# unitaryai/VTC

Measured on AMD Instinct MI355X. Metric: video-text pairs encoded/sec (config 3: 8-frame TimeSformer video + title + 5 comments, CAM) + 10k x 10k sim+R@K ms, higher is better.
Workload: dtype bf16 (video tower) + f16 (text tower blocks), fp32 accumulate; 1 GPU; configs/pretrained_clip_timesformer_comments_attention.jsonc PretrainedCLIP_TimeSformer_finaltf forward: 1024 pairs/GPU/step = 1024 videos (8 x 3 x 224 x 224) + 1024 titles + 5120 comments (77 tokens) + CAM + sim; pairs_per_gpu=1024, frames=8, text_tower=ragged: tokens after EOT are not computed, identical outputs, parallelism=dp1 (one process per GPU, no collective in the encode path)

## Files before the change

include/vtc_hip.h:

```cpp
#ifndef VTC_HIP_H
#define VTC_HIP_H

#include <stddef.h>
#include <stdint.h>

#ifdef __cplusplus
extern "C" {
#endif

enum { VTC_F32 = 0, VTC_BF16 = 1, VTC_U8 = 2 ,
       VTC_F16 = 3  };

enum { VTC_ACT_NONE = 0, VTC_ACT_NORMALIZE = 1, VTC_ACT_SQUASH = 2, VTC_ACT_TANH = 3,
       VTC_ACT_SUB_MEAN = 4, VTC_ACT_BN = 5 };

enum { VTC_SWEEP_F32 = 0,
       VTC_SWEEP_BF16X3 = 1,
       VTC_SWEEP_BF16 = 2,
       VTC_SWEEP_EXACT = 3 };

typedef struct {
  const float *ln1_g, *ln1_b;
  const void  *qkv_w;  const float *qkv_b;
  const void  *out_w;  const float *out_b;
  const float *ln2_g, *ln2_b;
  const void  *fc_w;   const float *fc_b;
  const void  *proj_w; const float *proj_b;
  const float *lnt_g, *lnt_b;
  const void  *tqkv_w; const float *tqkv_b;
  const void  *tout_w; const float *tout_b;
  const void  *tfc_w;  const float *tfc_b;
  const void  *qkv_wf;  const float *qkv_s,  *qkv_c;
  const void  *fc_wf;   const float *fc_s,   *fc_c;
  const void  *tqkv_wf; const float *tqkv_s, *tqkv_c;
} vtc_block_w;

enum { VTC_TOWER_NO_LN_FOLD = 1,
       VTC_TOWER_FULL_LAST_LAYER = 8,
       VTC_TOWER_NO_SPLITK = 16         };

typedef struct {
  int width, heads, layers, patch, grid, embed_dim, nframes;
  int variant;
  int flags;
  float pix_mean[3], pix_std[3];
  const void  *conv_w;
  const float *class_embedding;
  const float *pos;
  const float *temporal;
  const float *ln_pre_g, *ln_pre_b, *ln_post_g, *ln_post_b;
  const float *proj_t;
  const vtc_block_w *blocks;
} vtc_vision_w;

typedef struct {
  int width, heads, layers, ctx, vocab, embed_dim;
  int half_layers;
  int flags;
  const float *tok_emb;
  const float *pos;
  const float *ln_final_g, *ln_final_b;
  const float *proj_t;
  const vtc_block_w *blocks;
} vtc_text_w;

typedef struct {
  int width, heads, layers;
  int init_from_avg;
  int residual_activation;
  float squash_scale;
  const void  *final_linear;
  const float *mask_embedding;
  const vtc_block_w *blocks;
  const float *bn_mean, *bn_var;
  int flags;
} vtc_cam_w;
enum { VTC_CAM_NO_FUSED = 1 };

const char *vtc_last_error(void);
int vtc_abi_version(void);


size_t vtc_vision_workspace_bytes(const vtc_vision_w *w, int n_items, int frames, int dtype);
int vtc_vision_forward(const vtc_vision_w *w, const void *pixels, int pixel_dtype, int n_items, int frames,
                       float *out, void *ws, size_t ws_bytes, int dtype, void *stream);

size_t vtc_text_workspace_bytes(const vtc_text_w *w, int n_seq, int dtype);
int vtc_text_forward(const vtc_text_w *w, const int64_t *ids, int n_seq, float *out, void *ws, size_t ws_bytes,
                     int dtype, void *stream);

int vtc_text_forward2(const vtc_text_w *w, const int64_t *ids_a, int n_a, const int64_t *ids_b, int n_b, int ragged, float *out,
                      void *ws, size_t ws_bytes, int dtype, void *stream);

size_t vtc_text_ragged_workspace_bytes(const vtc_text_w *w, int n_seq, int total_rows, int dtype);
int vtc_text_forward_ragged(const vtc_text_w *w, const int64_t *ids, int n_seq, const int *seq_offsets, int total_rows,
                            float *out, void *ws, size_t ws_bytes, int dtype, void *stream);

size_t vtc_cam_workspace_bytes(const vtc_cam_w *w, int B, int nc, int dtype);
int vtc_cam_forward(const vtc_cam_w *w, const float *main_feats, const float *comm_feats, const int64_t *comments,
                    int ctx, int B, int nc, float *adapted, void *ws, size_t ws_bytes, int dtype, void *stream);
int vtc_cam_fused_gave_up(int device);

size_t vtc_cam_aux_workspace_bytes(const vtc_cam_w *w, int B, int nc, int na, int dtype);
int vtc_cam_forward_aux(const vtc_cam_w *w, const float *main_feats, const float *comm_feats, const int64_t *comments,
                        const float *aux, int ctx, int B, int nc, int na, float *adapted, void *ws, size_t ws_bytes, int dtype,
                        void *stream);

size_t vtc_feature_mlp_workspace_bytes(int n, int d);
int vtc_feature_mlp(const float *x, int n, int d, const float *w1, const float *b1, const float *w2, const float *b2, float *y,
                    void *ws, size_t ws_bytes, void *stream);


size_t vtc_resize_plan_bytes(int in_h, int in_w, int size);
int vtc_resize_plan(int in_h, int in_w, int size, void *plan_host, size_t bytes);
int vtc_resize_crop_u8(const unsigned char *frames, int n, int in_h, int in_w, int layout, const void *plan_dev, int size,
                       unsigned char *out, void *stream);

int vtc_normalize_rows(const float *x, float *out, int n, int d, void *stream);
int vtc_normalize_rows2(const float *x, float *outx, int nx, const float *y, float *outy, int ny, int d, int *flag, void *stream);
int vtc_mean_groups(const float *x, float *out, int n_groups, int group, int d, void *stream);
int vtc_pack_tokens(const int *tokens, const int *offsets, int n_seq, int ctx, int sot, int eot, int64_t *ids, void *stream);

int vtc_mean_head_groups(const float *a, const float *b, float *out, int n_groups, int group, int d, void *stream);
int vtc_segment_mean(const float *x, const int *offsets, float *out, int n_groups, int d, void *stream);
int vtc_nonfinite_flag(const float *x, size_t n, int *flag, void *stream);
int vtc_nonfinite_flag2(const float *x, size_t n, const float *y, size_t m, int *flag, void *stream);
int vtc_similarity(const float *v, const float *t, int nv, int nt, int d, const float *logit_scale, float *sim,
                   void *stream);

size_t vtc_clip_loss_workspace_bytes(int n);
int vtc_clip_loss(const float *sim, int n, float *loss, void *ws, size_t ws_bytes, void *stream);


size_t vtc_l2_topk_workspace_bytes(int n_gallery, int n_queries, int d, int precision, int rows_per_block);
int vtc_l2_topk(const float *gallery, const float *queries, int n_gallery, int n_queries, int d, int depth,
                int precision, int rows_per_block, int64_t *ids, float *dists, void *ws, size_t ws_bytes,
                void *stream);

size_t vtc_l2_topk_bidir_workspace_bytes(int n_a, int n_b, int d, int precision, int rows_per_block);
int vtc_l2_topk_bidir(const float *a, const float *b, int n_a, int n_b, int d, int depth, int precision, int rows_per_block,
                      int64_t *ids_b2a, float *dists_b2a, int64_t *ids_a2b, float *dists_a2b, void *ws, size_t ws_bytes,
                      void *stream);
int vtc_l2_sweep_row_block(void);
int vtc_l2_sweep_shard_supported(int n_total, int n_local, int depth);
size_t vtc_l2_sweep_shard_workspace_bytes(int n_total, int n_local, int d);
int vtc_l2_sweep_shard_rows(const float *a_all, const float *b_local, int n_total, int n_local, int d, int depth, int64_t *ids,
                            float *dists, unsigned *col_planes, int nblk_pad, void *ws, size_t ws_bytes, void *stream);
int vtc_l2_sweep_shard_cols(const float *b_all, const float *a_local, int n_total, int n_local, int d, int depth,
                            const unsigned *planes, int n_src, int nblk_pad, const int *src_base, int64_t *ids, float *dists,
                            void *ws, size_t ws_bytes, void *stream);
size_t vtc_l2_search_workspace_bytes(int n_gallery, int n_queries, int d, int depth);
int vtc_l2_search(const float *gallery, const float *queries, int n_gallery, int n_queries, int d, int depth, int64_t id_base,
                  int64_t *ids, float *dists, int *nonfinite, void *ws, size_t ws_bytes, void *stream);
int vtc_l2_search_masked(const float *gallery, const float *queries, const uint32_t *live, int n_gallery, int n_queries, int d, int depth,
                         int64_t id_base, int64_t *ids, float *dists, int *nonfinite, void *ws, size_t ws_bytes, void *stream);
int vtc_row_mask_pack(const uint8_t *flags, int n_rows, const uint32_t *and_mask, uint32_t *words, void *stream);
int vtc_l2_search_merge(const int64_t *ids_parts, const double *dists_parts, int n_parts, int n_queries, int depth, int64_t *ids,
                        float *dists, void *stream);
size_t vtc_l2_search_grouped_workspace_bytes(int n_gallery, int n_queries, int d, int depth);
int vtc_l2_search_grouped(const float *gallery, const float *queries, const uint32_t *live, const int32_t *groups, int n_gallery, int n_queries,
                          int d, int depth, int64_t id_base, int64_t *ids, int32_t *out_groups, float *dists, int *nonfinite, void *ws,
                          size_t ws_bytes, void *stream);
int vtc_l2_search_merge_grouped(const int64_t *ids_parts, const double *dists_parts, const int32_t *groups_parts, int n_parts, int n_queries,
                                int depth, int64_t *ids, int32_t *out_groups, float *dists, void *stream);
int vtc_recall_hits(const int64_t *ids, int n_queries, int depth, int64_t target_offset, const int *k_vals_host,
                    int nk, long long *hits, void *stream);
#define VTC_RECALL_NONFINITE (1ll << 40)
int vtc_l2_recall_bidir_supported(int n, int d);
size_t vtc_l2_recall_bidir_workspace_bytes(int n, int d);
int vtc_l2_recall_bidir(const float *a, const float *b, int n, int d, const int *k_vals_host, int nk, long long *hits_b_from_a,
                        long long *hits_a_from_b, void *ws, size_t ws_bytes, void *stream);
float vtc_l2_rank_kappa(int d);
size_t vtc_l2_rank_bidir_workspace_bytes(int n, int d, int rows_per_block, int reach_capacity);
int vtc_l2_rank_bidir(const float *a, const float *b, int n, int d, int rows_per_block, int reach_capacity, int64_t *rank_a,
                      int64_t *rank_b, int *nonfinite, void *ws, size_t ws_bytes, void *stream);
size_t vtc_l2_rank_shard_workspace_bytes(int n_total, int n_local, int d, int rows_per_block, int reach_capacity);
int vtc_l2_rank_shard(const float *a_all, const float *b_all, int n_total, int row_base, int n_local, int d, int rows_per_block,
                      int reach_capacity, int64_t *rank_a_local , int64_t *rank_b_part , int *nonfinite,
                      void *ws, size_t ws_bytes, void *stream);
size_t vtc_l2_rank_grouped_workspace_bytes(int n, int m, int d, int rows_per_block, int reach_capacity);
int vtc_l2_rank_grouped(const float *a, const float *b, const int *off, int n, int m, int d, int rows_per_block, int reach_capacity,
                        int64_t *rank_a , int64_t *rank_b , int *nonfinite, void *ws, size_t ws_bytes, void *stream);
size_t vtc_l2_rank_grouped_vunit_workspace_bytes(int n, int m, int d, int rows_per_block, int reach_capacity);
int vtc_l2_rank_grouped_vunit(const float *a, const float *b, const int *off, int n, int m, int d, int rows_per_block, int reach_capacity,
                              int64_t *rank_a , int64_t *rank_b , int64_t *rank_v , int *nonfinite, void *ws,
                              size_t ws_bytes, void *stream);
int vtc_l2_recall_shard_supported(int n_total, int n_local, int d);
int vtc_l2_recall_planes(const int *k_vals_host, int nk, int n_total);
int vtc_l2_recall_shard_rows(const float *a_all, const float *b_local, int n_total, int n_local, int row_base, int d,
                             const int *k_vals_host, int nk, long long *hits_b_from_a, unsigned *col_planes, int nblk_pad, void *ws,
                             size_t ws_bytes, void *stream);
int vtc_l2_recall_shard_cols(const float *b_all, const float *a_local, int n_total, int n_local, int row_base, int d,
                             const int *k_vals_host, int nk, const unsigned *planes, int n_src, int nblk_pad, const int *src_bounds,
                             long long *hits_a_from_b, void *ws, size_t ws_bytes, void *stream);
int vtc_recall_hits_pair(const int64_t *ids_a, const int64_t *ids_b, int n_queries, int depth, int64_t target_offset,
                         const int *k_vals_host, int nk, long long *hits_a, long long *hits_b, void *stream);

enum { VTC_EPI_STORE = 0,
       VTC_EPI_GELU = 1,
       VTC_EPI_RESID = 2 };
int vtc_gemm(const void *A, const void *W, const float *bias, void *out, int M, int N, int K, int dtype,
             int epilogue, int out_dtype, int skip_mod, void *stream);
size_t vtc_gemm_resid_layernorm_workspace_bytes(int M);
int vtc_gemm_resid_layernorm_supported(int M, int N, int K, int dtype);
int vtc_gemm_resid_layernorm(const void *A, const void *W, const float *bias, float *out, int M, int N, int K, int dtype,
                             int skip_mod, const float *ln_g, const float *ln_b, void *ln_out, void *ws, size_t ws_bytes,
                             void *stream);
int vtc_layernorm(const float *x, const float *g, const float *b, void *y, int rows, int width, int out_dtype,
                  const int *row_index, int row_mul, void *stream);
int vtc_attention(const void *qkv, void *out, float *cls_out, int n_seq, int L, int heads, int causal, int s2, int a0,
                  int a1, int a2, int a3, int pstride, int dtype, void *stream);

int vtc_single_query_attention(const void *qkv, const void *q, float *out, int n_out, int L, int heads, int s2, int a0, int a1, int a2,
                               int a3, int pstride, const int *eot, const int *offs, int ctx, int dtype, void *stream);

int vtc_transpose_f32(const float *x, float *y, int rows, int cols, void *stream);
int vtc_colsum_f32(const float *x, float *out, int rows, int cols, void *stream);
int vtc_layernorm_bwd(const float *x, const float *gamma, const float *dy, float *dx, float *dgamma, float *dbeta, int rows,
                      int width, int accumulate_dx, void *stream);
int vtc_attention_small_bwd(const float *qkv, const float *dout, float *dqkv, int n_seq, int L, int heads, void *stream);
int vtc_quickgelu(const float *x, const float *dy, float *out, size_t n, void *stream);
int vtc_normalize_rows_bwd(const float *x, const float *dy, float *dx, int n, int d, void *stream);
int vtc_clip_loss_bwd(const float *sim, int n, float *dsim, void *ws, size_t ws_bytes, void *stream);
int vtc_adam_step(float *p, const float *g, float *m, float *v, float *vmax, size_t n, float lr, float beta1, float beta2,
                  float eps, int step, int amsgrad, void *stream);
int vtc_axpby(float *out, const float *x, const float *y, float a, float b, size_t n, void *stream);
int vtc_scale_rows(float *x, const float *s, int rows, int d, int group, void *stream);

enum { VTC_PROF_GEMM_BF16 = 0, VTC_PROF_GEMM_F32 = 1, VTC_PROF_ATTN = 2, VTC_PROF_NORM = 3, VTC_PROF_EMBED = 4,
       VTC_PROF_TOPK = 5, VTC_PROF_NCLASS = 6 };
enum { VTC_PROF_REGION_OTHER = 0, VTC_PROF_REGION_ATTN = 1, VTC_PROF_REGION_MLP = 2, VTC_PROF_NREGION = 3 };
int vtc_prof_begin(void);
int vtc_prof_end(void *stream, double *ms, long long *launches, double *work);
int vtc_prof_end_regions(void *stream, double *ms, long long *launches, double *work);
int vtc_prof_end_records(void *stream, int max, int *n, int *cls, int *region, double *ms, double *work, int *tag);
long long vtc_debug_launch_count(void);

#ifdef __cplusplus
}
#endif
#endif
```

vtc_amd/_lib.py:

```python
from __future__ import annotations

import ctypes as C
import os

_HERE = os.path.dirname(os.path.abspath(__file__))
LIB_PATH = os.environ.get("VTC_HIP_LIB") or os.path.join(_HERE, "lib", "libvtc_hip.so")

VTC_F32, VTC_BF16, VTC_U8 = 0, 1, 2
ACT_NONE, ACT_NORMALIZE, ACT_SQUASH, ACT_TANH, ACT_SUB_MEAN, ACT_BN = 0, 1, 2, 3, 4, 5
SWEEP_F32, SWEEP_BF16X3, SWEEP_BF16, SWEEP_EXACT = 0, 1, 2, 3
EPI_STORE, EPI_GELU, EPI_RESID = 0, 1, 2
PROF_CLASSES = ("gemm_bf16", "gemm_f32", "attention", "norm", "embed", "topk")
PROF_REGIONS = ("other", "attn", "mlp")
VTC_F16 = 3
TOWER_NO_LN_FOLD, TOWER_FULL_LAST_LAYER, TOWER_NO_SPLITK = 1, 8, 16
CAM_NO_FUSED = 1
RECALL_NONFINITE = 1 << 40
ABI_VERSION = 7

vp, fp, ip = C.c_void_p, C.c_void_p, C.c_void_p


class BlockW(C.Structure):
    _fields_ = [(n, C.c_void_p) for n in (
        "ln1_g", "ln1_b", "qkv_w", "qkv_b", "out_w", "out_b", "ln2_g", "ln2_b", "fc_w", "fc_b", "proj_w", "proj_b",
        "lnt_g", "lnt_b", "tqkv_w", "tqkv_b", "tout_w", "tout_b", "tfc_w", "tfc_b",
        "qkv_wf", "qkv_s", "qkv_c", "fc_wf", "fc_s", "fc_c", "tqkv_wf", "tqkv_s", "tqkv_c")]


class VisionW(C.Structure):
    _fields_ = [("width", C.c_int), ("heads", C.c_int), ("layers", C.c_int), ("patch", C.c_int), ("grid", C.c_int),
                ("embed_dim", C.c_int), ("nframes", C.c_int), ("variant", C.c_int), ("flags", C.c_int),
                ("pix_mean", C.c_float * 3), ("pix_std", C.c_float * 3),
                ("conv_w", C.c_void_p), ("class_embedding", C.c_void_p), ("pos", C.c_void_p), ("temporal", C.c_void_p),
                ("ln_pre_g", C.c_void_p), ("ln_pre_b", C.c_void_p), ("ln_post_g", C.c_void_p), ("ln_post_b", C.c_void_p),
                ("proj_t", C.c_void_p), ("blocks", C.POINTER(BlockW))]


class TextW(C.Structure):
    _fields_ = [("width", C.c_int), ("heads", C.c_int), ("layers", C.c_int), ("ctx", C.c_int), ("vocab", C.c_int),
                ("embed_dim", C.c_int), ("half_layers", C.c_int), ("flags", C.c_int),
                ("tok_emb", C.c_void_p), ("pos", C.c_void_p), ("ln_final_g", C.c_void_p), ("ln_final_b", C.c_void_p),
                ("proj_t", C.c_void_p), ("blocks", C.POINTER(BlockW))]


class CamW(C.Structure):
    _fields_ = [("width", C.c_int), ("heads", C.c_int), ("layers", C.c_int), ("init_from_avg", C.c_int),
                ("residual_activation", C.c_int), ("squash_scale", C.c_float),
                ("final_linear", C.c_void_p), ("mask_embedding", C.c_void_p), ("blocks", C.POINTER(BlockW)),
                ("bn_mean", C.c_void_p), ("bn_var", C.c_void_p), ("flags", C.c_int)]


SIGNATURES = {
    "vtc_last_error": (C.c_char_p, []),
    "vtc_abi_version": (C.c_int, []),
    "vtc_vision_workspace_bytes": (C.c_size_t, [C.POINTER(VisionW), C.c_int, C.c_int, C.c_int]),
    "vtc_vision_forward": (C.c_int, [C.POINTER(VisionW), vp, C.c_int, C.c_int, C.c_int, fp, vp, C.c_size_t, C.c_int, vp]),
    "vtc_text_workspace_bytes": (C.c_size_t, [C.POINTER(TextW), C.c_int, C.c_int]),
    "vtc_text_forward": (C.c_int, [C.POINTER(TextW), ip, C.c_int, fp, vp, C.c_size_t, C.c_int, vp]),
    "vtc_text_forward2": (C.c_int, [C.POINTER(TextW), ip, C.c_int, ip, C.c_int, C.c_int, fp, vp, C.c_size_t, C.c_int, vp]),
    "vtc_text_ragged_workspace_bytes": (C.c_size_t, [C.POINTER(TextW), C.c_int, C.c_int, C.c_int]),
    "vtc_text_forward_ragged": (C.c_int, [C.POINTER(TextW), ip, C.c_int, ip, C.c_int, fp, vp, C.c_size_t, C.c_int, vp]),
    "vtc_cam_workspace_bytes": (C.c_size_t, [C.POINTER(CamW), C.c_int, C.c_int, C.c_int]),
    "vtc_cam_forward": (C.c_int, [C.POINTER(CamW), fp, fp, ip, C.c_int, C.c_int, C.c_int, fp, vp, C.c_size_t, C.c_int, vp]),
    "vtc_cam_fused_gave_up": (C.c_int, [C.c_int]),
    "vtc_cam_aux_workspace_bytes": (C.c_size_t, [C.POINTER(CamW), C.c_int, C.c_int, C.c_int, C.c_int]),
    "vtc_cam_forward_aux": (C.c_int, [C.POINTER(CamW), fp, fp, ip, fp, C.c_int, C.c_int, C.c_int, C.c_int, fp, vp, C.c_size_t, C.c_int,
                                      vp]),
    "vtc_feature_mlp_workspace_bytes": (C.c_size_t, [C.c_int, C.c_int]),
    "vtc_feature_mlp": (C.c_int, [fp, C.c_int, C.c_int, fp, fp, fp, fp, fp, vp, C.c_size_t, vp]),
    "vtc_resize_plan_bytes": (C.c_size_t, [C.c_int, C.c_int, C.c_int]),
    "vtc_resize_plan": (C.c_int, [C.c_int, C.c_int, C.c_int, vp, C.c_size_t]),
    "vtc_resize_crop_u8": (C.c_int, [vp, C.c_int, C.c_int, C.c_int, C.c_int, vp, C.c_int, vp, vp]),
    "vtc_normalize_rows": (C.c_int, [fp, fp, C.c_int, C.c_int, vp]),
    "vtc_normalize_rows2": (C.c_int, [fp, fp, C.c_int, fp, fp, C.c_int, C.c_int, vp, vp]),
    "vtc_mean_groups": (C.c_int, [fp, fp, C.c_int, C.c_int, C.c_int, vp]),
    "vtc_nonfinite_flag": (C.c_int, [fp, C.c_size_t, vp, vp]),
    "vtc_nonfinite_flag2": (C.c_int, [fp, C.c_size_t, fp, C.c_size_t, vp, vp]),
    "vtc_mean_head_groups": (C.c_int, [fp, fp, fp, C.c_int, C.c_int, C.c_int, vp]),
    "vtc_pack_tokens": (C.c_int, [vp, vp, C.c_int, C.c_int, C.c_int, C.c_int, vp, vp]),
    "vtc_single_query_attention": (C.c_int, [vp, vp, fp] + [C.c_int] * 9 + [vp, vp, C.c_int, C.c_int, vp]),
    "vtc_segment_mean": (C.c_int, [fp, ip, fp, C.c_int, C.c_int, vp]),
    "vtc_similarity": (C.c_int, [fp, fp, C.c_int, C.c_int, C.c_int, fp, fp, vp]),
    "vtc_clip_loss_workspace_bytes": (C.c_size_t, [C.c_int]),
    "vtc_clip_loss": (C.c_int, [fp, C.c_int, fp, vp, C.c_size_t, vp]),
    "vtc_l2_topk_workspace_bytes": (C.c_size_t, [C.c_int, C.c_int, C.c_int, C.c_int, C.c_int]),
    "vtc_l2_topk": (C.c_int, [fp, fp, C.c_int, C.c_int, C.c_int, C.c_int, C.c_int, C.c_int, ip, fp, vp, C.c_size_t, vp]),
    "vtc_l2_topk_bidir_workspace_bytes": (C.c_size_t, [C.c_int, C.c_int, C.c_int, C.c_int, C.c_int]),
    "vtc_l2_topk_bidir": (C.c_int, [fp, fp, C.c_int, C.c_int, C.c_int, C.c_int, C.c_int, C.c_int, ip, fp, ip, fp, vp, C.c_size_t, vp]),
    "vtc_l2_sweep_row_block": (C.c_int, []),
    "vtc_l2_sweep_shard_supported": (C.c_int, [C.c_int, C.c_int, C.c_int]),
    "vtc_l2_sweep_shard_workspace_bytes": (C.c_size_t, [C.c_int, C.c_int, C.c_int]),
    "vtc_l2_sweep_shard_rows": (C.c_int, [fp, fp, C.c_int, C.c_int, C.c_int, C.c_int, ip, fp, vp, C.c_int, vp, C.c_size_t, vp]),
    "vtc_l2_sweep_shard_cols": (C.c_int, [fp, fp, C.c_int, C.c_int, C.c_int, C.c_int, vp, C.c_int, C.c_int, vp, ip, fp, vp,
                                          C.c_size_t, vp]),
    "vtc_l2_search_workspace_bytes": (C.c_size_t, [C.c_int, C.c_int, C.c_int, C.c_int]),
    "vtc_l2_search": (C.c_int, [fp, fp, C.c_int, C.c_int, C.c_int, C.c_int, C.c_int64, ip, fp, ip, vp, C.c_size_t, vp]),
    "vtc_l2_search_masked": (C.c_int, [fp, fp, ip, C.c_int, C.c_int, C.c_int, C.c_int, C.c_int64, ip, fp, ip, vp, C.c_size_t, vp]),
    "vtc_row_mask_pack": (C.c_int, [vp, C.c_int, ip, ip, vp]),
    "vtc_l2_search_merge": (C.c_int, [ip, fp, C.c_int, C.c_int, C.c_int, ip, fp, vp]),
    "vtc_l2_search_grouped_workspace_bytes": (C.c_size_t, [C.c_int, C.c_int, C.c_int, C.c_int]),
    "vtc_l2_search_grouped": (C.c_int, [fp, fp, ip, ip, C.c_int, C.c_int, C.c_int, C.c_int, C.c_int64, ip, ip, fp, ip, vp, C.c_size_t, vp]),
    "vtc_l2_search_merge_grouped": (C.c_int, [ip, fp, ip, C.c_int, C.c_int, C.c_int, ip, ip, fp, vp]),
    "vtc_recall_hits": (C.c_int, [ip, C.c_int, C.c_int, C.c_int64, C.POINTER(C.c_int), C.c_int, vp, vp]),
    "vtc_recall_hits_pair": (C.c_int, [ip, ip, C.c_int, C.c_int, C.c_int64, C.POINTER(C.c_int), C.c_int, vp, vp, vp]),
    "vtc_l2_recall_bidir_supported": (C.c_int, [C.c_int, C.c_int]),
    "vtc_l2_recall_bidir_workspace_bytes": (C.c_size_t, [C.c_int, C.c_int]),
    "vtc_l2_recall_bidir": (C.c_int, [fp, fp, C.c_int, C.c_int, C.POINTER(C.c_int), C.c_int, ip, ip, vp, C.c_size_t, vp]),
    "vtc_l2_rank_kappa": (C.c_float, [C.c_int]),
    "vtc_l2_rank_bidir_workspace_bytes": (C.c_size_t, [C.c_int, C.c_int, C.c_int, C.c_int]),
    "vtc_l2_rank_bidir": (C.c_int, [fp, fp, C.c_int, C.c_int, C.c_int, C.c_int, ip, ip, ip, vp, C.c_size_t, vp]),
    "vtc_l2_rank_shard_workspace_bytes": (C.c_size_t, [C.c_int, C.c_int, C.c_int, C.c_int, C.c_int]),
    "vtc_l2_rank_shard": (C.c_int, [fp, fp, C.c_int, C.c_int, C.c_int, C.c_int, C.c_int, C.c_int, ip, ip, ip, vp, C.c_size_t, vp]),
    "vtc_l2_rank_grouped_workspace_bytes": (C.c_size_t, [C.c_int, C.c_int, C.c_int, C.c_int, C.c_int]),
    "vtc_l2_rank_grouped": (C.c_int, [fp, fp, ip, C.c_int, C.c_int, C.c_int, C.c_int, C.c_int, ip, ip, ip, vp, C.c_size_t, vp]),
    "vtc_l2_rank_grouped_vunit_workspace_bytes": (C.c_size_t, [C.c_int, C.c_int, C.c_int, C.c_int, C.c_int]),
    "vtc_l2_rank_grouped_vunit": (C.c_int, [fp, fp, ip, C.c_int, C.c_int, C.c_int, C.c_int, C.c_int, ip, ip, ip, ip, vp, C.c_size_t, vp]),
    "vtc_l2_recall_shard_supported": (C.c_int, [C.c_int, C.c_int, C.c_int]),
    "vtc_l2_recall_planes": (C.c_int, [C.POINTER(C.c_int), C.c_int, C.c_int]),
    "vtc_l2_recall_shard_rows": (C.c_int, [fp, fp, C.c_int, C.c_int, C.c_int, C.c_int, C.POINTER(C.c_int), C.c_int, ip, vp, C.c_int, vp, C.c_size_t, vp]),
    "vtc_l2_recall_shard_cols": (C.c_int, [fp, fp, C.c_int, C.c_int, C.c_int, C.c_int, C.POINTER(C.c_int), C.c_int, vp, C.c_int, C.c_int, vp, ip, vp,
                                           C.c_size_t, vp]),
    "vtc_gemm": (C.c_int, [vp, vp, fp, vp, C.c_int, C.c_int, C.c_int, C.c_int, C.c_int, C.c_int, C.c_int, vp]),
    "vtc_gemm_resid_layernorm_workspace_bytes": (C.c_size_t, [C.c_int]),
    "vtc_gemm_resid_layernorm_supported": (C.c_int, [C.c_int, C.c_int, C.c_int, C.c_int]),
    "vtc_gemm_resid_layernorm": (C.c_int, [vp, vp, fp, fp, C.c_int, C.c_int, C.c_int, C.c_int, C.c_int, fp, fp, vp, vp, C.c_size_t, vp]),
    "vtc_layernorm": (C.c_int, [fp, fp, fp, vp, C.c_int, C.c_int, C.c_int, ip, C.c_int, vp]),
    "vtc_prof_begin": (C.c_int, []),
    "vtc_prof_end": (C.c_int, [vp, C.POINTER(C.c_double), C.POINTER(C.c_longlong), C.POINTER(C.c_double)]),
    "vtc_prof_end_regions": (C.c_int, [vp, C.POINTER(C.c_double), C.POINTER(C.c_longlong), C.POINTER(C.c_double)]),
    "vtc_prof_end_records": (C.c_int, [vp, C.c_int, C.POINTER(C.c_int), C.POINTER(C.c_int), C.POINTER(C.c_int), C.POINTER(C.c_double),
                                       C.POINTER(C.c_double), C.POINTER(C.c_int)]),
    "vtc_debug_launch_count": (C.c_longlong, []),
    "vtc_attention": (C.c_int, [vp, vp, fp, C.c_int, C.c_int, C.c_int, C.c_int, C.c_int, C.c_int, C.c_int, C.c_int,
                                C.c_int, C.c_int, C.c_int, vp]),
    "vtc_transpose_f32": (C.c_int, [fp, fp, C.c_int, C.c_int, vp]),
    "vtc_colsum_f32": (C.c_int, [fp, fp, C.c_int, C.c_int, vp]),
    "vtc_layernorm_bwd": (C.c_int, [fp, fp, fp, fp, fp, fp, C.c_int, C.c_int, C.c_int, vp]),
    "vtc_attention_small_bwd": (C.c_int, [fp, fp, fp, C.c_int, C.c_int, C.c_int, vp]),
    "vtc_quickgelu": (C.c_int, [fp, fp, fp, C.c_size_t, vp]),
    "vtc_normalize_rows_bwd": (C.c_int, [fp, fp, fp, C.c_int, C.c_int, vp]),
    "vtc_clip_loss_bwd": (C.c_int, [fp, C.c_int, fp, vp, C.c_size_t, vp]),
    "vtc_adam_step": (C.c_int, [fp, fp, fp, fp, fp, C.c_size_t, C.c_float, C.c_float, C.c_float, C.c_float, C.c_int, C.c_int, vp]),
    "vtc_axpby": (C.c_int, [fp, fp, fp, C.c_float, C.c_float, C.c_size_t, vp]),
    "vtc_scale_rows": (C.c_int, [fp, fp, C.c_int, C.c_int, C.c_int, vp]),
}

_lib = None


def lib() -> C.CDLL:
    global _lib
    if _lib is None:
        if not os.path.exists(LIB_PATH):
            raise RuntimeError(
                f"libvtc_hip.so not found at {LIB_PATH}: build it with `python -c 'import __graft_entry__ as g; g.build()'` "
                "(or `make -C vtc_amd/csrc`).  vtc_amd has no CPU or PyTorch fallback.")
        l = C.CDLL(LIB_PATH)
        for name, (res, args) in SIGNATURES.items():
            f = getattr(l, name)
            f.restype, f.argtypes = res, args
        _lib = l
    return _lib


def check(rc: int, what: str):
    if rc != 0:
        msg = lib().vtc_last_error().decode("utf-8", "replace")
        raise RuntimeError(f"{what} failed: {msg}")
```

vtc_amd/csrc/common.h:

```cpp
#pragma once
#include <hip/hip_runtime.h>
#include <stdint.h>
#include <stdio.h>

#include "../../include/vtc_hip.h"

typedef unsigned short bf16_t;
typedef __attribute__((ext_vector_type(8))) short bf16x8;
typedef __attribute__((ext_vector_type(4))) short bf16x4;
typedef __attribute__((ext_vector_type(4))) float f32x4;
typedef __attribute__((ext_vector_type(16))) float f32x16;

#define VTC_WAVE 64

void vtc_count_launch();
#undef hipLaunchKernelGGL
#define hipLaunchKernelGGL(kernelName, numBlocks, numThreads, memPerBlock, streamId, ...)             \
  do {                                                                                              \
    vtc_count_launch();                                                                             \
    (kernelName)<<<(numBlocks), (numThreads), (memPerBlock), (streamId)>>>(__VA_ARGS__);            \
  } while (0)

void vtc_set_error(const char *fmt, ...);

#define VTC_CHECK(cond, ...)          \
  do {                                \
    if (!(cond)) {                    \
      vtc_set_error(__VA_ARGS__);     \
      return 1;                       \
    }                                 \
  } while (0)

#define VTC_LAUNCH_CHECK(name)                                                  \
  do {                                                                          \
    hipError_t e_ = hipGetLastError();                                          \
    if (e_ != hipSuccess) {                                                     \
      vtc_set_error("%s: launch failed: %s", name, hipGetErrorString(e_));      \
      return 1;                                                                 \
    }                                                                           \
  } while (0)

#define VTC_LAUNCH_CHECK2(fn, stage)                                                          \
  do {                                                                                        \
    hipError_t e_ = hipGetLastError();                                                        \
    if (e_ != hipSuccess) {                                                                   \
      vtc_set_error("%s %s: launch failed: %s", fn, stage, hipGetErrorString(e_));            \
      return 1;                                                                               \
    }                                                                                         \
  } while (0)

__device__ __forceinline__ bf16_t f2bf(float f) {
  __bf16 b = (__bf16)f;
  return __builtin_bit_cast(bf16_t, b);
}
__device__ __forceinline__ float bf2f(bf16_t b) {
  return __builtin_bit_cast(float, ((unsigned)b) << 16);
}

struct f16_t { unsigned short v; };
typedef __attribute__((ext_vector_type(8))) _Float16 f16x8;
__device__ __forceinline__ unsigned short f2h(float f) {
  _Float16 h = (_Float16)f;
  return __builtin_bit_cast(unsigned short, h);
}
__device__ __forceinline__ float h2f(unsigned short b) { return (float)__builtin_bit_cast(_Float16, b); }
template <typename T> __device__ __forceinline__ unsigned short cvt16(float f);
template <> __device__ __forceinline__ unsigned short cvt16<bf16_t>(float f) { return f2bf(f); }
template <> __device__ __forceinline__ unsigned short cvt16<f16_t>(float f) { return f2h(f); }

template <typename T> __device__ __forceinline__ unsigned pack16(float a, float b);
template <> __device__ __forceinline__ unsigned pack16<bf16_t>(float a, float b) {
  typedef float f2v_t __attribute__((ext_vector_type(2)));
  typedef __bf16 bf2v_t __attribute__((ext_vector_type(2)));
  return __builtin_bit_cast(unsigned, __builtin_convertvector((f2v_t){a, b}, bf2v_t));
}
template <> __device__ __forceinline__ unsigned pack16<f16_t>(float a, float b) {
  typedef float f2v_t __attribute__((ext_vector_type(2)));
  typedef _Float16 h2v_t __attribute__((ext_vector_type(2)));
  return __builtin_bit_cast(unsigned, __builtin_convertvector((f2v_t){a, b}, h2v_t));
}

template <typename T> __device__ __forceinline__ float up16(unsigned short b);
template <> __device__ __forceinline__ float up16<bf16_t>(unsigned short b) { return __builtin_bit_cast(float, ((unsigned)b) << 16); }
template <> __device__ __forceinline__ float up16<f16_t>(unsigned short b) { return h2f(b); }

template <typename T> struct ElemOps;
template <> struct ElemOps<float> {
  static constexpr int kDtype = VTC_F32;
  __device__ static __forceinline__ float load(const float *p) { return *p; }
  __device__ static __forceinline__ void store(float *p, float v) { *p = v; }
  __device__ static __forceinline__ void store4(float *p, float a, float b, float c, float d) {
    *reinterpret_cast<float4 *>(p) = make_float4(a, b, c, d);
  }
  __device__ static __forceinline__ float4 load4(const float *p) { return *reinterpret_cast<const float4 *>(p); }
};
template <> struct ElemOps<bf16_t> {
  static constexpr int kDtype = VTC_BF16;
  __device__ static __forceinline__ float load(const bf16_t *p) { return bf2f(*p); }
  __device__ static __forceinline__ void store(bf16_t *p, float v) { *p = f2bf(v); }
  __device__ static __forceinline__ void store4(bf16_t *p, float a, float b, float c, float d) {
    ushort4 v;
    v.x = f2bf(a); v.y = f2bf(b); v.z = f2bf(c); v.w = f2bf(d);
    *reinterpret_cast<ushort4 *>(p) = v;
  }
  __device__ static __forceinline__ float4 load4(const bf16_t *p) {
    ushort4 v = *reinterpret_cast<const ushort4 *>(p);
    return make_float4(bf2f(v.x), bf2f(v.y), bf2f(v.z), bf2f(v.w));
  }
};

template <> struct ElemOps<f16_t> {
  static constexpr int kDtype = VTC_F16;
  __device__ static __forceinline__ float load(const f16_t *p) { return h2f(p->v); }
  __device__ static __forceinline__ void store(f16_t *p, float v) { p->v = f2h(v); }
  __device__ static __forceinline__ void store4(f16_t *p, float a, float b, float c, float d) {
    ushort4 v;
    v.x = f2h(a); v.y = f2h(b); v.z = f2h(c); v.w = f2h(d);
    *reinterpret_cast<ushort4 *>(p) = v;
  }
  __device__ static __forceinline__ float4 load4(const f16_t *p) {
    ushort4 v = *reinterpret_cast<const ushort4 *>(p);
    return make_float4(h2f(v.x), h2f(v.y), h2f(v.z), h2f(v.w));
  }
};

__device__ __forceinline__ float wave_sum(float v) {
#pragma unroll
  for (int o = 32; o > 0; o >>= 1) v += __shfl_xor(v, o, 64);
  return v;
}
__device__ __forceinline__ float wave_max(float v) {
#pragma unroll
  for (int o = 32; o > 0; o >>= 1) v = fmaxf(v, __shfl_xor(v, o, 64));
  return v;
}

__device__ __forceinline__ auto permlane16_swap(unsigned a, unsigned b) { return __builtin_amdgcn_permlane16_swap(a, b, false, false); }
__device__ __forceinline__ unsigned xor32_of(unsigned x, bool upper) {
  const auto r = __builtin_amdgcn_permlane32_swap(x, x, false, false);
  return upper ? r[0] : r[1];
}
__device__ __forceinline__ unsigned xor16_of(unsigned x, bool odd_row) {
  const auto r = permlane16_swap(x, x);
  return odd_row ? r[0] : r[1];
}

static inline size_t align_up(size_t x, size_t a) { return (x + a - 1) / a * a; }
constexpr int cdiv(int a, int b) { return (a + b - 1) / b; }

struct Bump {
  char *base;
  size_t off = 0;
  explicit Bump(void *b) : base((char *)b) {}
  void *take(size_t bytes) {
    const size_t o = off;
    off = align_up(off + bytes, 256);
    return base ? base + o : nullptr;
  }
};

#include <atomic>
struct PerDeviceOnce {
  std::atomic<unsigned long long> done{0};
};
inline int ensure_dynamic_lds(PerDeviceOnce &once, const void *kernel, int bytes, const char *name) {
  int dev = 0;
  if (hipGetDevice(&dev) != hipSuccess || dev < 0 || dev >= 64) dev = 0;
  const unsigned long long bit = 1ull << dev;
  if (once.done.load(std::memory_order_acquire) & bit) return 0;
  const hipError_t e = hipFuncSetAttribute(kernel, hipFuncAttributeMaxDynamicSharedMemorySize, bytes);
  if (e != hipSuccess) {
    vtc_set_error("%s: hipFuncSetAttribute(MaxDynamicSharedMemorySize = %d) failed on device %d: %s", name, bytes, dev,
                  hipGetErrorString(e));
    return 1;
  }
  once.done.fetch_or(bit, std::memory_order_release);
  return 0;
}

struct ProfScope {
  ProfScope(int cls, double work, hipStream_t s, const int *m_dev = nullptr);
  ~ProfScope();
  void tag(int a, int b, int c);
  hipStream_t stream_;
  int idx_;
};

struct ProfRegion {
  explicit ProfRegion(int region);
  ~ProfRegion();
  int prev_;
};

struct GemmEpi {
  int mode = VTC_EPI_STORE;
  int out_dtype = VTC_F32;
  int skip_mod = 0;
  const float *pos = nullptr;
  const float *temporal = nullptr;
  int P = 0, F = 0, T = 0;
  int frames_major = 0;
  int gather = 0, grid = 0, res = 0, patch = 0;
  const float *rown = nullptr;
  const float *coln = nullptr;
  const float *scale_log = nullptr;
  int ldo = 0;
  unsigned *rowk = nullptr, *colk = nullptr;
  int nblk_c = 0, nblk_r = 0;
  const float *ln_g = nullptr, *ln_b = nullptr;
  void *ln_out = nullptr;
  int *ln_cnt = nullptr;
  void *y16 = nullptr;
  void *y16lo = nullptr;
  float *fold_part = nullptr;
  const float *fold_stat = nullptr, *fold_s = nullptr;
  const int *m_dev = nullptr;
  int ksplit = 0, split_stride = 0;
};
enum { EPI_PATCH = 3, EPI_L2DIST = 4, EPI_SCALE = 5, EPI_L2MIN = 6, EPI_RESID_LN = 7,
       EPI_FOLD_BASE = 8, EPI_STORE_FOLD = 8, EPI_GELU_FOLD = 9, EPI_RESID_FOLD = 10,
       EPI_RESID_FOLD_C = 11 ,
       EPI_L2MIN2 = 12 ,
       EPI_L2MIN3 = 13  };
#define VTC_L2MIN_INF 0x7F800000u
#define L2MIN_PLANES 4
constexpr int l2min_row_planes(int mode) { return (mode == EPI_L2MIN2 || mode == EPI_L2MIN3) ? 2 : L2MIN_PLANES; }
constexpr int l2min_col_planes(int mode) { return mode == EPI_L2MIN2 ? 2 : (mode == EPI_L2MIN3 ? 3 : L2MIN_PLANES); }
constexpr bool l2min_half_keys(int mode) { return mode == EPI_L2MIN2 || mode == EPI_L2MIN3; }

int launch_gemm(const void *A, const void *W, const float *bias, void *out, int M, int N, int K, int dtype,
                const GemmEpi &epi, hipStream_t stream);
namespace vtcgemm { int num_cus(); }
bool gemm_resid_ln_supported(int M, int N, int K, int dtype);
bool gemm_patch_gather_supported(int n_frames, int grid, int patch, int res, int pixel_dtype, int dtype);
int launch_layernorm(const float *x, const float *g, const float *b, void *y, int rows, int width, int out_dtype,
                     const int *row_index, int row_mul, bool no_norm, hipStream_t stream, const int *rows_dev = nullptr);
int launch_fold_stats(const float *part, int nb, int rows, float *stat, hipStream_t stream, const int *rows_dev = nullptr);
int launch_ln_cast_rowstats(const float *x, const float *gamma, const float *beta, void *y16, void *y16lo, float *stat, int rows, int width, int dtype,
                            hipStream_t stream);
int launch_splitk_resid_rows(const float *part, int nsl, int stride, const float *bias, void *hi, void *lo, float *stat, int rows, int width, int dtype,
                             hipStream_t stream, const int *rows_dev = nullptr);
int launch_cast_rowstats(const float *x, void *y16, void *y16lo, float *stat, int rows, int width, int dtype, hipStream_t stream,
                         const int *rows_dev = nullptr);
int launch_gather_rows(const void *src, void *dst, int n, int row_bytes, const int *row_index, int row_mul, hipStream_t stream);
int launch_split_merge_rows(const void *hi, const void *lo, float *x, int n, int width, const int *row_index, int row_mul, int dtype,
                            hipStream_t stream, const int *rows_dev = nullptr);
struct TextIds {
  const int64_t *a, *b;
  int n_a, n_b;
  __host__ __device__ const int64_t *row(int s, int ctx) const { return s < n_a ? a + (size_t)s * ctx : b + (size_t)(s - n_a) * ctx; }
};
int launch_single_query_attention(const void *qkv, const void *q, float *out, int n_out, int L, int heads, int s2, int a0, int a1, int a2,
                                  int a3, int pstride, const int *eot, const int *offs, int ctx, int dtype, hipStream_t stream);
int launch_mean_cast(const float *x, void *out, int n, int F, int W, int dtype, hipStream_t stream);
int launch_attention(const void *qkv, void *out, float *cls_out, int n_seq, int L, int heads, int causal, int s2,
                     int a0, int a1, int a2, int a3, int pstride, int dtype, hipStream_t stream);
```

vtc_amd/csrc/towers.hip:

```cpp
#include <stdarg.h>
#include <string.h>

#include "common.h"

static thread_local char g_err[512] = "";
void vtc_set_error(const char *fmt, ...) {
  va_list ap;
  va_start(ap, fmt);
  vsnprintf(g_err, sizeof(g_err), fmt, ap);
  va_end(ap);
}
extern "C" const char *vtc_last_error(void) { return g_err; }
extern "C" int vtc_abi_version(void) { return 7; }
int launch_im2row(const void *px, int pixel_dtype, void *out, int dtype, int n_frames, int grid, int patch, int res, const float *mean, const float *stdv, hipStream_t stream);
int patch_k_padded(int patch);
int launch_pixels_u8_to_operand(const void *px, void *out, int dtype, int n_frames, int res, const float *mean, const float *stdv, hipStream_t stream);
int launch_cls_rows(float *x, const float *cls, const float *pos0, int n_items, int T, int W, hipStream_t stream);
int launch_cls_mean(const float *cls_tmp, void *out, int dtype, int n_items, int F, int T, int W, hipStream_t stream);
int launch_text_prep(const TextIds &ids, int n_seq, int ctx, int *lens, int *offsets, int *m_dev, hipStream_t stream);
int launch_text_embed(const TextIds &ids, const float *tok, const float *pos, float *x, int *eot_row, int n_seq, int ctx, int W, int vocab, hipStream_t stream);
int launch_text_embed_ragged(const TextIds &ids, const float *tok, const float *pos, const int *seq_offsets, float *x, int *eot_row, int n_seq, int ctx, int W, int vocab, hipStream_t stream);
int launch_text_embed_ragged_pair(const TextIds &ids, const float *tok, const float *pos, const int *seq_offsets, void *y16, void *y16lo, float *stat, int *eot_row, int n_seq, int ctx, int W, int vocab, int dtype, hipStream_t stream);
int launch_attention_ragged(const void *qkv, void *out, int n_seq, int max_L, int heads, int causal, const int *seq_offsets, double flops, const int *rows_dev, int dtype, hipStream_t stream);
int launch_attention_generic_small(const void *qkv, void *out, int n_seq, int L, int heads, int hd, int dtype, hipStream_t stream);
int launch_cam_tokens(const float *main_f, const float *comm, const int64_t *comments, const float *mask_emb, const float *aux, float *X, int B, int nc, int na, int ctx, int D, hipStream_t stream);
int launch_cls_global_attention(const void *qkv, void *out, int n_items, int Ttok, int heads, int dtype, hipStream_t stream);
int launch_cam_finalize(const float *Y, const float *lin, const float *main_f, float *out, int B, int Lc, int D, int init_from_avg, int act, float scale, const float *bn_mean, const float *bn_var, hipStream_t stream);

bool cam_fused_supported(const vtc_cam_w *w, int B, int nc, int na, int dtype);
size_t cam_fused_bar_bytes();
int launch_cam_fused(const vtc_cam_w *w, const float *main_feats, const float *comm_feats, const int64_t *comments, const float *aux, int ctx,
                     int B, int nc, int na, float *adapted, float *x, float *big, float *att, int *bar, hipStream_t stream);
namespace {


#define RUN(call)        \
  do {                   \
    int rc_ = (call);    \
    if (rc_) return rc_; \
  } while (0)

inline int esz(int dtype) { return dtype == VTC_F32 ? 4 : 2; }

int gemm(const void *A, const void *W, const float *bias, void *out, int M, int N, int K, int dtype, int mode, int out_dtype, hipStream_t s) {
  GemmEpi e;
  e.mode = mode; e.out_dtype = out_dtype;
  return launch_gemm(A, W, bias, out, M, N, K, dtype, e, s);
}

struct Fold {
  bool on = false;
  void *xb = nullptr;
  void *xl = nullptr;
  float *part = nullptr;
  float *stat = nullptr;
  int rows_pad = 0;
  int fmt = -1;
  float *splitk = nullptr;
};
constexpr int SPLITK_MAX = 4, SPLITK_MAX_ROWS = 1024;
inline int splitk_slices(int rows_pad, int W, int K) {
  if (rows_pad > SPLITK_MAX_ROWS || K < 2048 || W % 256 != 0 || W > 1024) return 1;
  const long tiles = (long)(rows_pad / 64) * (W / 64);
  for (int s = SPLITK_MAX; s >= 2; --s)
    if (K % (64 * s) == 0 && K / s >= 256 && tiles * s <= 2L * vtcgemm::num_cus()) return s;
  return 1;
}
inline int pad256(int rows) { return (rows + 255) / 256 * 256; }
void plan_fold(Bump &b, Fold &f, size_t rows, int W, int dtype) {
  if (dtype == VTC_F32) return;
  f.rows_pad = (int)rows;
  f.xb = b.take(rows * W * 2);
  f.xl = b.take(rows * W * 2);
  f.part = (float *)b.take((size_t)(W / 64 + 1) * rows * 8);
  f.stat = (float *)b.take(rows * 8);
  if (rows <= (size_t)SPLITK_MAX_ROWS) f.splitk = (float *)b.take((size_t)SPLITK_MAX * rows * W * 4);
}

struct Rows {
  int n;
  const int *dev = nullptr;
  Rows(int n_) : n(n_) {}
  Rows(int n_, const int *dev_) : n(n_), dev(dev_) {}
  const int *dev_pad() const { return dev ? dev + 1 : nullptr; }
};

struct Act {
  float *x = nullptr;
  void *h = nullptr, *big = nullptr;
  Fold fold;
  Rows rows = 0;
  int W = 0;
  hipStream_t s = nullptr;
};
void plan_act(Bump &b, Act &a, size_t rows, int W, size_t big_elems, int dtype, hipStream_t s) {
  a.W = W; a.s = s;
  a.x = (float *)b.take(rows * W * 4);
  a.h = b.take(rows * W * esz(dtype));
  a.big = b.take(big_elems * esz(dtype));
}
void fold_begin(Act &a, const vtc_block_w *blocks, int layers, int dtype, bool timesformer, int flags) {
  if (flags & VTC_TOWER_NO_SPLITK) a.fold.splitk = nullptr;
  a.fold.on = !(flags & VTC_TOWER_NO_LN_FOLD) && dtype != VTC_F32 && a.W % 256 == 0;
  for (int l = 0; l < layers; ++l)
    if (!blocks[l].qkv_wf || !blocks[l].fc_wf || (timesformer && !blocks[l].tqkv_wf)) a.fold.on = false;
}

int fold_merge_rows(Act &a, int n, const int *row_index, int row_mul) {
  if (!a.fold.on || a.fold.fmt < 0) return 0;
  return launch_split_merge_rows(a.fold.xb, a.fold.xl, a.x, n, a.W, row_index, row_mul, a.fold.fmt, a.s);
}

int fold_enter(Act &a, int dtype) {
  Fold &f = a.fold;
  if (f.fmt == dtype) return 0;
  if (f.fmt >= 0) RUN(launch_split_merge_rows(f.xb, f.xl, a.x, a.rows.n, a.W, nullptr, 1, f.fmt, a.s, a.rows.dev));
  RUN(launch_cast_rowstats(a.x, f.xb, f.xl, f.stat, a.rows.n, a.W, dtype, a.s, a.rows.dev));
  f.fmt = dtype;
  return 0;
}

struct Proj { const float *g, *bt; const void *w; const float *bias; const void *wf; const float *s, *c; };
inline Proj qkv_of(const vtc_block_w &b) { return {b.ln1_g, b.ln1_b, b.qkv_w, b.qkv_b, b.qkv_wf, b.qkv_s, b.qkv_c}; }
inline Proj tqkv_of(const vtc_block_w &b) { return {b.lnt_g, b.lnt_b, b.tqkv_w, b.tqkv_b, b.tqkv_wf, b.tqkv_s, b.tqkv_c}; }
inline Proj fc_of(const vtc_block_w &b) { return {b.ln2_g, b.ln2_b, b.fc_w, b.fc_b, b.fc_wf, b.fc_s, b.fc_c}; }

int ln_proj(Act &a, Proj p, int N, int dtype, int mode, int col0 = 0, int ncols = 0) {
  const int W = a.W;
  void *out = a.big;
  GemmEpi e;
  e.mode = mode; e.out_dtype = dtype; e.ldo = N;
  if (ncols > 0) {
    const size_t wo = (size_t)col0 * W * esz(dtype);
    p.w = (const char *)p.w + wo;
    if (p.wf) p.wf = (const char *)p.wf + wo;
    if (p.bias) p.bias += col0;
    if (p.s) p.s += col0;
    if (p.c) p.c += col0;
    out = (char *)out + (size_t)col0 * esz(dtype);
    N = ncols;
  }
  if (!a.fold.on) {
    RUN(launch_layernorm(a.x, p.g, p.bt, a.h, a.rows.n, W, dtype, nullptr, 1, false, a.s, a.rows.dev));
    e.m_dev = a.rows.dev;
    return launch_gemm(a.h, p.w, p.bias, out, a.rows.n, N, W, dtype, e, a.s);
  }
  RUN(fold_enter(a, dtype));
  e.fold_stat = a.fold.stat; e.fold_s = p.s; e.m_dev = a.rows.dev_pad();
  return launch_gemm(a.fold.xb, p.wf, p.c, out, a.fold.rows_pad, N, W, dtype, e, a.s);
}

int resid_proj(Act &a, const void *A, const void *w, const float *bias, int K, int dtype, int skip_mod, bool center = false) {
  const int W = a.W;
  Fold &f = a.fold;
  const int *m_dev = f.on ? a.rows.dev_pad() : a.rows.dev;
  GemmEpi e;
  e.mode = VTC_EPI_RESID; e.out_dtype = VTC_F32; e.skip_mod = skip_mod; e.m_dev = m_dev;
  if (!f.on) return launch_gemm(A, w, bias, a.x, a.rows.n, W, K, dtype, e, a.s);
  RUN(fold_enter(a, dtype));
  const int nsl = (center && skip_mod == 0 && f.splitk) ? splitk_slices(f.rows_pad, W, K) : 1;
  if (nsl > 1) {
    GemmEpi ek;
    ek.mode = VTC_EPI_STORE; ek.out_dtype = VTC_F32; ek.m_dev = m_dev; ek.ksplit = nsl; ek.split_stride = f.rows_pad * W;
    RUN(launch_gemm(A, w, nullptr, f.splitk, f.rows_pad, W, K, dtype, ek, a.s));
    return launch_splitk_resid_rows(f.splitk, nsl, f.rows_pad * W, bias, f.xb, f.xl, f.stat, f.rows_pad, W, dtype, a.s, m_dev);
  }
  e.y16 = f.xb; e.y16lo = f.xl; e.fold_part = f.part;
  if (center) e.fold_stat = f.stat;
  RUN(launch_gemm(A, w, bias, a.x, f.rows_pad, W, K, dtype, e, a.s));
  return launch_fold_stats(f.part, W / 64, f.rows_pad, f.stat, a.s, m_dev);
}

int mlp_part(Act &a, const vtc_block_w &b, int dtype) {
  ProfRegion region(VTC_PROF_REGION_MLP);
  RUN(ln_proj(a, fc_of(b), 4 * a.W, dtype, VTC_EPI_GELU));
  return resid_proj(a, a.big, b.proj_w, b.proj_b, 4 * a.W, dtype, 0, true);
}

int attn_part_contig(Act &a, const vtc_block_w &b, int n_seq, int L, int heads, int causal, int dtype) {
  const int W = a.W;
  ProfRegion region(VTC_PROF_REGION_ATTN);
  RUN(ln_proj(a, qkv_of(b), 3 * W, dtype, VTC_EPI_STORE));
  if (W != heads * 64) {
    VTC_CHECK(!causal && W % heads == 0, "attention: head_dim %d/%d", W, heads);
    RUN(launch_attention_generic_small(a.big, a.h, n_seq, L, heads, W / heads, dtype, a.s));
  } else {
    RUN(launch_attention(a.big, a.h, nullptr, n_seq, L, heads, causal, 1, 0, L, 0, 0, 1, dtype, a.s));
  }
  return resid_proj(a, a.h, b.out_w, b.out_b, W, dtype, 0);
}

enum class LastBlock { AllRows, OutputRowsAfterAttention, OneQueryPerSequence };
inline LastBlock last_block_path(int flags, int layers, bool variant1) {
  if ((flags & VTC_TOWER_FULL_LAST_LAYER) || layers == 0) return LastBlock::AllRows;
  return variant1 ? LastBlock::OutputRowsAfterAttention : LastBlock::OneQueryPerSequence;
}
struct Tail {
  float *x = nullptr;
  void *a = nullptr;
  void *h = nullptr;
  void *big = nullptr;
  float *sq = nullptr;
};
void plan_tail(Bump &b, Tail &t, int n, int W) {
  t.x = (float *)b.take((size_t)n * W * 4);
  t.a = b.take((size_t)n * W * 4);
  t.h = b.take((size_t)n * W * 4);
  t.big = b.take((size_t)n * 4 * W * 4);
  t.sq = (float *)b.take((size_t)n * W * 4);
}
int gather_output_rows(Act &a, Tail &t, int n, const int *row_index, int row_mul) {
  RUN(fold_merge_rows(a, n, row_index, row_mul));
  return launch_gather_rows(a.x, t.x, n, a.W * 4, row_index, row_mul, a.s);
}
int tail_query(Act &a, const vtc_block_w &b, Tail &t, int n, const int *row_index, int row_mul, int dtype) {
  RUN(gather_output_rows(a, t, n, row_index, row_mul));
  RUN(launch_layernorm(t.x, b.ln1_g, b.ln1_b, t.h, n, a.W, dtype, nullptr, 1, false, a.s));
  return gemm(t.h, b.qkv_w, b.qkv_b, t.big, n, a.W, a.W, dtype, VTC_EPI_STORE, dtype, a.s);
}
int tail_finish(const vtc_block_w &b, Tail &t, int n, int W, int dtype, hipStream_t s) {
  RUN(gemm(t.a, b.out_w, b.out_b, t.x, n, W, W, dtype, VTC_EPI_RESID, VTC_F32, s));
  Act ta{t.x, t.h, t.big, Fold(), n, W, s};
  return mlp_part(ta, b, dtype);
}

struct VisionWs {
  Act a;
  float *cls_tmp;
  void *lnp;
  Tail tail;
  size_t total;
};
VisionWs plan_vision(const vtc_vision_w *w, int n_items, int F, int dtype, void *ws, hipStream_t s = nullptr) {
  Bump b(ws);
  VisionWs v;
  const int P = w->grid * w->grid, T = 1 + P * F, W = w->width;
  const size_t rows = (size_t)pad256(n_items * T);
  const size_t patch_elems = (size_t)n_items * F * P * patch_k_padded(w->patch);
  plan_act(b, v.a, rows, W, patch_elems > rows * 4 * W ? patch_elems : rows * 4 * W, dtype, s);
  v.a.rows = n_items * T;
  v.cls_tmp = (float *)b.take((size_t)n_items * (F > P ? F : P) * W * 4);
  v.lnp = b.take((size_t)n_items * W * 4);
  plan_fold(b, v.a.fold, rows, W, dtype);
  plan_tail(b, v.tail, n_items, W);
  v.total = b.off;
  return v;
}

struct TextWs {
  Act a;
  void *lnp;
  int *eot;
  int *lens, *offs, *mdev;
  Tail tail;
  size_t total;
};
TextWs plan_text(int rows_, int n_seq, int W, int dtype, void *ws, hipStream_t s = nullptr) {
  Bump b(ws);
  TextWs t;
  const size_t rows = (size_t)pad256(rows_);
  plan_act(b, t.a, rows, W, rows * 4 * W, dtype, s);
  t.a.rows = rows_;
  t.lnp = b.take((size_t)n_seq * W * 4);
  t.eot = (int *)b.take((size_t)n_seq * 4);
  t.lens = (int *)b.take((size_t)n_seq * 4);
  t.offs = (int *)b.take((size_t)(n_seq + 1) * 4);
  t.mdev = (int *)b.take(16);
  plan_fold(b, t.a.fold, rows, W, dtype);
  plan_tail(b, t.tail, n_seq, W);
  t.total = b.off;
  return t;
}

}

extern "C" size_t vtc_vision_workspace_bytes(const vtc_vision_w *w, int n_items, int frames, int dtype) {
  return plan_vision(w, n_items, frames, dtype, nullptr).total;
}

extern "C" int vtc_vision_forward(const vtc_vision_w *w, const void *pixels, int pixel_dtype, int n_items, int F, float *out,
                                  void *ws, size_t ws_bytes, int dtype, void *stream_) {
  hipStream_t s = (hipStream_t)stream_;
  VTC_CHECK(w && pixels && out && ws, "vision_forward: null argument");
  VTC_CHECK(dtype == VTC_F32 || dtype == VTC_BF16 || dtype == VTC_F16, "vision_forward: bad dtype %d", dtype);
  VTC_CHECK(n_items > 0 && F > 0, "vision_forward: n_items=%d frames=%d", n_items, F);
  const bool tsf = w->nframes > 0, v1 = w->variant == 1;
  VTC_CHECK(tsf || F == 1, "vision_forward: the image tower takes frames == 1 (got %d)", F);
  VTC_CHECK(!tsf || F <= w->nframes, "vision_forward: %d frames > temporal_embed rows %d", F, w->nframes);
  VTC_CHECK(w->width == w->heads * 64, "vision_forward: head_dim must be 64 (width %d, heads %d)", w->width, w->heads);
  const int P = w->grid * w->grid, T = 1 + P * F, W = w->width;
  VTC_CHECK(1 + P <= 272 && F <= 272, "vision_forward: sequence too long (1+P=%d, F=%d; the attention cores cover 272 tokens)", 1 + P, F);
  VTC_CHECK(w->variant == 0 || w->variant == 1, "vision_forward: unknown variant %d", w->variant);
  VTC_CHECK(!(w->variant == 1 && w->nframes == 0), "vision_forward: variant 1 (model/timesformer_clip.py) is a video tower: nframes must be > 0");
  const int rows = n_items * T, res = w->grid * w->patch;
  VisionWs v = plan_vision(w, n_items, F, dtype, ws, s);
  VTC_CHECK(ws_bytes >= v.total, "vision_forward: workspace too small (%zu < %zu)", ws_bytes, v.total);
  Act &a = v.a;

  VTC_CHECK(pixel_dtype == VTC_F32 || pixel_dtype == VTC_BF16 || pixel_dtype == VTC_U8 || pixel_dtype == VTC_F16, "vision_forward: bad pixel dtype %d", pixel_dtype);
  {
    GemmEpi e;
    e.mode = EPI_PATCH; e.out_dtype = VTC_F32; e.pos = w->pos; e.temporal = tsf ? w->temporal : nullptr;
    e.P = P; e.F = F; e.T = T; e.ldo = W; e.frames_major = v1;
    const void *act = a.big;
    const bool few = (long)n_items * F * P < 4096;
    if (!few && gemm_patch_gather_supported(n_items * F, w->grid, w->patch, res, pixel_dtype, dtype) && ((size_t)pixels & 15) == 0) {
      e.gather = 1; e.grid = w->grid; e.res = res; e.patch = w->patch;
      act = pixels;
    } else if (!few && pixel_dtype == VTC_U8 && gemm_patch_gather_supported(n_items * F, w->grid, w->patch, res, dtype, dtype) && ((size_t)pixels & 15) == 0) {
      RUN(launch_pixels_u8_to_operand(pixels, a.big, dtype, n_items * F, res, w->pix_mean, w->pix_std, s));
      e.gather = 1; e.grid = w->grid; e.res = res; e.patch = w->patch;
    } else {
      RUN(launch_im2row(pixels, pixel_dtype, a.big, dtype, n_items * F, w->grid, w->patch, res, w->pix_mean, w->pix_std, s));
    }
    RUN(launch_gemm(act, w->conv_w, nullptr, a.x, n_items * F * P, W, patch_k_padded(w->patch), dtype, e, s));
  }
  RUN(launch_cls_rows(a.x, w->class_embedding, w->pos, n_items, T, W, s));
  fold_begin(a, w->blocks, w->layers, dtype, tsf, w->flags);
  if (a.fold.on && w->layers > 0) {
    RUN(launch_ln_cast_rowstats(a.x, w->ln_pre_g, w->ln_pre_b, a.fold.xb, a.fold.xl, a.fold.stat, rows, W, dtype, s));
    a.fold.fmt = dtype;
  } else {
    RUN(launch_layernorm(a.x, w->ln_pre_g, w->ln_pre_b, a.x, rows, W, VTC_F32, nullptr, 1, false, s));
  }

  auto v1_attention = [&](const vtc_block_w &b) -> int {
    RUN(ln_proj(a, tqkv_of(b), 3 * W, dtype, VTC_EPI_STORE));
    RUN(launch_attention(a.big, a.h, v.cls_tmp, n_items * P, 1 + F, w->heads, 0, P, 0, T, 0, 1, P, dtype, s));
    RUN(launch_cls_global_attention(a.big, a.h, n_items, T, w->heads, dtype, s));
    RUN(resid_proj(a, a.h, b.tout_w, b.tout_b, W, dtype, 0));
    RUN(ln_proj(a, qkv_of(b), 3 * W, dtype, VTC_EPI_STORE));
    RUN(launch_attention(a.big, a.h, v.cls_tmp, n_items * F, 1 + P, w->heads, 0, F, 0, T, 0, P, 1, dtype, s));
    return launch_cls_global_attention(a.big, a.h, n_items, T, w->heads, dtype, s);
  };
  auto time_branch = [&](const vtc_block_w &b) -> int {
    RUN(ln_proj(a, tqkv_of(b), 3 * W, dtype, VTC_EPI_STORE));
    RUN(launch_attention(a.big, a.h, nullptr, n_items * P, F, w->heads, 0, P, 1, T, F, 0, 1, dtype, s));
    if (b.tout_w) {
      RUN(gemm(a.h, b.tout_w, b.tout_b, a.big, a.fold.on ? a.fold.rows_pad : rows, W, W, dtype, VTC_EPI_STORE, dtype, s));
      return resid_proj(a, a.big, b.tfc_w, b.tfc_b, W, dtype, T);
    }
    return resid_proj(a, a.h, b.tfc_w, b.tfc_b, W, dtype, T);
  };

  const LastBlock last = last_block_path(w->flags, w->layers, v1);
  for (int l = 0; l < w->layers; ++l) {
    const vtc_block_w &b = w->blocks[l];
    ProfRegion region(VTC_PROF_REGION_ATTN);
    switch (l == w->layers - 1 ? last : LastBlock::AllRows) {
      case LastBlock::AllRows:
        if (v1) {
          RUN(v1_attention(b));
          RUN(resid_proj(a, a.h, b.out_w, b.out_b, W, dtype, 0));
        } else if (tsf) {
          RUN(time_branch(b));
          RUN(ln_proj(a, qkv_of(b), 3 * W, dtype, VTC_EPI_STORE));
          RUN(launch_attention(a.big, a.h, v.cls_tmp, n_items * F, 1 + P, w->heads, 0, F, 0, T, 0, 1, F, dtype, s));
          RUN(launch_cls_mean(v.cls_tmp, a.h, dtype, n_items, F, T, W, s));
          RUN(resid_proj(a, a.h, b.out_w, b.out_b, W, dtype, 0));
        } else {
          RUN(attn_part_contig(a, b, n_items, T, w->heads, 0, dtype));
        }
        RUN(mlp_part(a, b, dtype));
        break;
      case LastBlock::OutputRowsAfterAttention:
        RUN(v1_attention(b));
        RUN(gather_output_rows(a, v.tail, n_items, nullptr, T));
        RUN(launch_gather_rows(a.h, v.tail.a, n_items, W * esz(dtype), nullptr, T, s));
        RUN(tail_finish(b, v.tail, n_items, W, dtype, s));
        break;
      case LastBlock::OneQueryPerSequence:
        if (tsf) RUN(time_branch(b));
        RUN(tail_query(a, b, v.tail, n_items, nullptr, T, dtype));
        RUN(ln_proj(a, qkv_of(b), 3 * W, dtype, VTC_EPI_STORE, W, 2 * W));
        RUN(launch_single_query_attention(a.big, v.tail.big, v.cls_tmp, n_items * F, 1 + P, w->heads, F, 0, T, 0, tsf ? 1 : 0, F, nullptr, nullptr, 0, dtype, s));
        RUN(launch_mean_cast(v.cls_tmp, v.tail.a, n_items, F, W, dtype, s));
        RUN(tail_finish(b, v.tail, n_items, W, dtype, s));
        break;
    }
  }
  if (last != LastBlock::AllRows) {
    RUN(launch_layernorm(v.tail.x, w->ln_post_g, w->ln_post_b, v.lnp, n_items, W, VTC_F32, nullptr, 1, false, s));
  } else {
    RUN(fold_merge_rows(a, n_items, nullptr, T));
    RUN(launch_layernorm(a.x, w->ln_post_g, w->ln_post_b, v.lnp, n_items, W, VTC_F32, nullptr, T, false, s));
  }
  RUN(gemm(v.lnp, w->proj_t, nullptr, out, n_items, w->embed_dim, W, VTC_F32, VTC_EPI_STORE, VTC_F32, s));
  return 0;
}

extern "C" size_t vtc_text_workspace_bytes(const vtc_text_w *w, int n_seq, int dtype) {
  return plan_text(n_seq * w->ctx, n_seq, w->width, dtype, nullptr).total;
}

namespace {
enum class TextRows { Dense, HostOffsets, DeviceOffsets };
int text_forward_impl(const vtc_text_w *w, const TextIds &ids, TextRows kind, const int *seq_offsets, int total_rows, float *out, void *ws,
                      size_t ws_bytes, int dtype, hipStream_t s, const char *who) {
  const int n_seq = ids.n_a + ids.n_b, W = w->width;
  VTC_CHECK(dtype == VTC_F32 || dtype == VTC_BF16 || dtype == VTC_F16, "%s: bad dtype %d", who, dtype);
  VTC_CHECK(w->ctx <= 80, "%s: context %d > 80 unsupported", who, w->ctx);
  VTC_CHECK(w->width == w->heads * 64, "%s: head_dim must be 64", who);
  const int rows_host = kind == TextRows::HostOffsets ? total_rows : n_seq * w->ctx;
  TextWs t = plan_text(rows_host, n_seq, W, dtype, ws, s);
  VTC_CHECK(ws_bytes >= t.total, "%s: workspace too small (%zu < %zu)", who, ws_bytes, t.total);
  Act &a = t.a;
  const int *offs = seq_offsets;
  if (kind == TextRows::DeviceOffsets) {
    RUN(launch_text_prep(ids, n_seq, w->ctx, t.lens, t.offs, t.mdev, s));
    offs = t.offs;
    a.rows = Rows(rows_host, t.mdev);
  }
  fold_begin(a, w->blocks, w->layers, dtype, false, w->flags);
  const LastBlock last = last_block_path(w->flags, w->layers, false);
  const bool ragged = kind != TextRows::Dense;
  const int dl0 = (dtype == VTC_BF16 && w->half_layers > 0) ? VTC_F16 : dtype;
  if (!ragged) {
    RUN(launch_text_embed(ids, w->tok_emb, w->pos, a.x, t.eot, n_seq, w->ctx, W, w->vocab, s));
  } else if (a.fold.on && (w->layers > 1 || (w->layers == 1 && last == LastBlock::AllRows))) {
    RUN(launch_text_embed_ragged_pair(ids, w->tok_emb, w->pos, offs, a.fold.xb, a.fold.xl, a.fold.stat, t.eot, n_seq, w->ctx, W, w->vocab, dl0, s));
    a.fold.fmt = dl0;
  } else {
    RUN(launch_text_embed_ragged(ids, w->tok_emb, w->pos, offs, a.x, t.eot, n_seq, w->ctx, W, w->vocab, s));
  }
  const double attn_flops_per_row = 4.0 * (0.5 * w->ctx) * 64 * w->heads;
  for (int l = 0; l < w->layers; ++l) {
    const vtc_block_w &b = w->blocks[l];
    const int dl = (dtype == VTC_BF16 && l < w->half_layers) ? VTC_F16 : dtype;
    ProfRegion region(VTC_PROF_REGION_ATTN);
    switch (l == w->layers - 1 ? last : LastBlock::AllRows) {
      case LastBlock::AllRows:
        if (kind == TextRows::Dense) {
          RUN(attn_part_contig(a, b, n_seq, w->ctx, w->heads, 1, dl));
        } else {
          RUN(ln_proj(a, qkv_of(b), 3 * W, dl, VTC_EPI_STORE));
          RUN(launch_attention_ragged(a.big, a.h, n_seq, w->ctx, w->heads, 1, offs, attn_flops_per_row * (a.rows.dev ? 1.0 : a.rows.n), a.rows.dev, dl, s));
          RUN(resid_proj(a, a.h, b.out_w, b.out_b, W, dl, 0));
        }
        RUN(mlp_part(a, b, dl));
        break;
      case LastBlock::OneQueryPerSequence:
        RUN(tail_query(a, b, t.tail, n_seq, t.eot, 1, dl));
        RUN(ln_proj(a, qkv_of(b), 3 * W, dl, VTC_EPI_STORE, W, 2 * W));
        RUN(launch_single_query_attention(a.big, t.tail.big, t.tail.sq, n_seq, 0, w->heads, 1, 0, 0, 0, 0, 1, t.eot,
                                          kind == TextRows::Dense ? nullptr : offs, w->ctx, dl, s));
        RUN(launch_mean_cast(t.tail.sq, t.tail.a, n_seq, 1, W, dl, s));
        RUN(tail_finish(b, t.tail, n_seq, W, dl, s));
        break;
      case LastBlock::OutputRowsAfterAttention: VTC_CHECK(false, "%s: last_block_path() chose the variant-1 video tower's path", who);
    }
  }
  if (last != LastBlock::AllRows) {
    RUN(launch_layernorm(t.tail.x, w->ln_final_g, w->ln_final_b, t.lnp, n_seq, W, VTC_F32, nullptr, 1, false, s));
  } else {
    RUN(fold_merge_rows(a, n_seq, t.eot, 1));
    RUN(launch_layernorm(a.x, w->ln_final_g, w->ln_final_b, t.lnp, n_seq, W, VTC_F32, t.eot, 1, false, s));
  }
  RUN(gemm(t.lnp, w->proj_t, nullptr, out, n_seq, w->embed_dim, W, VTC_F32, VTC_EPI_STORE, VTC_F32, s));
  return 0;
}
}

extern "C" int vtc_text_forward(const vtc_text_w *w, const int64_t *ids, int n_seq, float *out, void *ws, size_t ws_bytes,
                                int dtype, void *stream_) {
  VTC_CHECK(w && ids && out && ws, "text_forward: null argument");
  VTC_CHECK(n_seq > 0, "text_forward: n_seq=%d", n_seq);
  return text_forward_impl(w, TextIds{ids, nullptr, n_seq, 0}, TextRows::Dense, nullptr, 0, out, ws, ws_bytes, dtype, (hipStream_t)stream_,
                           "text_forward");
}

extern "C" int vtc_text_forward2(const vtc_text_w *w, const int64_t *ids_a, int n_a, const int64_t *ids_b, int n_b, int ragged,
                                 float *out, void *ws, size_t ws_bytes, int dtype, void *stream_) {
  VTC_CHECK(w && ids_a && out && ws && (ids_b || n_b == 0), "text_forward2: null argument");
  VTC_CHECK(n_a > 0 && n_b >= 0, "text_forward2: n_a=%d n_b=%d", n_a, n_b);
  return text_forward_impl(w, TextIds{ids_a, ids_b, n_a, n_b}, ragged ? TextRows::DeviceOffsets : TextRows::Dense, nullptr, 0, out, ws,
                           ws_bytes, dtype, (hipStream_t)stream_, "text_forward2");
}

extern "C" size_t vtc_text_ragged_workspace_bytes(const vtc_text_w *w, int n_seq, int total_rows, int dtype) {
  return plan_text(total_rows, n_seq, w->width, dtype, nullptr).total;
}

extern "C" int vtc_text_forward_ragged(const vtc_text_w *w, const int64_t *ids, int n_seq, const int *seq_offsets, int total_rows,
                                       float *out, void *ws, size_t ws_bytes, int dtype, void *stream_) {
  VTC_CHECK(w && ids && seq_offsets && out && ws, "text_forward_ragged: null argument");
  VTC_CHECK(n_seq > 0 && total_rows >= n_seq && total_rows <= n_seq * w->ctx, "text_forward_ragged: n_seq=%d total_rows=%d", n_seq, total_rows);
  return text_forward_impl(w, TextIds{ids, nullptr, n_seq, 0}, TextRows::HostOffsets, seq_offsets, total_rows, out, ws, ws_bytes, dtype,
                           (hipStream_t)stream_, "text_forward_ragged");
}

static size_t cam_ws_bytes(const vtc_cam_w *w, int B, int Lc, int dtype) {
  TextWs t = plan_text(B * Lc, B, w->width, dtype, nullptr);
  return t.total + align_up((size_t)B * w->width * 4, 256) + align_up(cam_fused_bar_bytes(), 256);
}

extern "C" size_t vtc_cam_workspace_bytes(const vtc_cam_w *w, int B, int nc, int dtype) { return cam_ws_bytes(w, B, 1 + nc, dtype); }

extern "C" size_t vtc_cam_aux_workspace_bytes(const vtc_cam_w *w, int B, int nc, int na, int dtype) {
  return cam_ws_bytes(w, B, 1 + nc + na, dtype);
}

static int cam_forward_impl(const vtc_cam_w *w, const float *main_feats, const float *comm_feats, const int64_t *comments, const float *aux,
                            int ctx, int B, int nc, int na, float *adapted, void *ws, size_t ws_bytes, int dtype, hipStream_t s) {
  VTC_CHECK(w && main_feats && comm_feats && comments && adapted && ws && (aux || na == 0), "cam_forward: null argument");
  VTC_CHECK(dtype == VTC_F32 || dtype == VTC_BF16, "cam_forward: bad dtype %d", dtype);
  VTC_CHECK(B > 0 && nc >= 0 && na >= 0 && 1 + nc + na <= 80, "cam_forward: B=%d nc=%d na=%d", B, nc, na);
  const int D = w->width, Lc = 1 + nc + na, rows = B * Lc;
  VTC_CHECK(w->heads >= 1 && w->width % w->heads == 0 && (w->width == w->heads * 64 || (w->width / w->heads <= 128 && Lc <= 16)),
            "cam_forward: head_dim %d / %d: 64, or <= 128 with at most 16 tokens per item", w->width, w->heads);
  TextWs t = plan_text(rows, B, D, dtype, ws, s);
  Act &a = t.a;
  float *lin = (float *)((char *)ws + t.total);
  VTC_CHECK(ws_bytes >= cam_ws_bytes(w, B, Lc, dtype), "cam_forward: workspace too small");
  if (cam_fused_supported(w, B, nc, na, dtype)) {
    const int rc = launch_cam_fused(w, main_feats, comm_feats, comments, aux, ctx, B, nc, na, adapted, a.x, (float *)a.big, (float *)a.h,
                                    (int *)((char *)ws + t.total + align_up((size_t)B * w->width * 4, 256)), s);
    if (rc >= 0) return rc;
  }
  RUN(launch_cam_tokens(main_feats, comm_feats, comments, w->mask_embedding, aux, a.x, B, nc, na, ctx, D, s));
  for (int l = 0; l < w->layers; ++l) {
    RUN(attn_part_contig(a, w->blocks[l], B, Lc, w->heads, 0, dtype));
    RUN(mlp_part(a, w->blocks[l], dtype));
  }
  if (!w->init_from_avg) {
    RUN(launch_layernorm(a.x, nullptr, nullptr, t.lnp, B, D, dtype, nullptr, Lc, true, s));
    RUN(gemm(t.lnp, w->final_linear, nullptr, lin, B, D, D, dtype, VTC_EPI_STORE, VTC_F32, s));
  }
  RUN(launch_cam_finalize(a.x, lin, main_feats, adapted, B, Lc, D, w->init_from_avg, w->residual_activation, w->squash_scale, w->bn_mean, w->bn_var, s));
  return 0;
}

extern "C" int vtc_cam_forward(const vtc_cam_w *w, const float *main_feats, const float *comm_feats, const int64_t *comments,
                               int ctx, int B, int nc, float *adapted, void *ws, size_t ws_bytes, int dtype, void *stream_) {
  return cam_forward_impl(w, main_feats, comm_feats, comments, nullptr, ctx, B, nc, 0, adapted, ws, ws_bytes, dtype, (hipStream_t)stream_);
}

extern "C" int vtc_cam_forward_aux(const vtc_cam_w *w, const float *main_feats, const float *comm_feats, const int64_t *comments,
                                   const float *aux, int ctx, int B, int nc, int na, float *adapted, void *ws, size_t ws_bytes, int dtype,
                                   void *stream_) {
  return cam_forward_impl(w, main_feats, comm_feats, comments, aux, ctx, B, nc, na, adapted, ws, ws_bytes, dtype, (hipStream_t)stream_);
}
```

vtc_amd/ops.py:

```python
from __future__ import annotations

import ctypes as C
import functools
from typing import Optional, Sequence

import torch

from . import _lib as L

_TDT = {torch.float32: L.VTC_F32, torch.bfloat16: L.VTC_BF16, torch.float16: L.VTC_F16}


def _stream() -> int:
    return torch.cuda.current_stream().cuda_stream


def on_device(fn):
    @functools.wraps(fn)
    def wrapped(*args, **kwargs):
        dev = None
        for a in args + tuple(kwargs.values()):
            if isinstance(a, torch.Tensor) and a.is_cuda:
                if dev is None:
                    dev = a.device
                elif a.device != dev:
                    raise RuntimeError(f"vtc_amd.{fn.__name__}: tensors on different devices ({dev} and {a.device})")
        if dev is None or dev.index == torch.cuda.current_device():
            return fn(*args, **kwargs)
        with torch.cuda.device(dev):
            return fn(*args, **kwargs)
    return wrapped


def _gpu(t: torch.Tensor, dtype=None, name="tensor") -> torch.Tensor:
    if not t.is_cuda:
        raise RuntimeError(f"vtc_amd: {name} must be on the GPU (got {t.device}); this package has no CPU path")
    if dtype is not None and t.dtype != dtype:
        raise TypeError(f"vtc_amd: {name} must be {dtype}, got {t.dtype}")
    return t if t.is_contiguous() else t.contiguous()


def dtype_code(dtype) -> int:
    if isinstance(dtype, int):
        return dtype
    return _TDT[dtype]


def torch_dtype(code: int):
    return {L.VTC_BF16: torch.bfloat16, L.VTC_F16: torch.float16}.get(code, torch.float32)


def workspace(nbytes: int, device) -> torch.Tensor:
    return torch.empty(max(int(nbytes), 256), dtype=torch.uint8, device=device)


def _ws_for(ws: Optional[torch.Tensor], need: int, device) -> torch.Tensor:
    return ws if ws is not None and ws.numel() >= need and ws.device == device else workspace(need, device)


def _k_array(k_vals: Sequence[int]):
    return (C.c_int * len(k_vals))(*[int(k) for k in k_vals])


@on_device
def gemm(a: torch.Tensor, w: torch.Tensor, bias: Optional[torch.Tensor] = None, epilogue: int = L.EPI_STORE,
         out: Optional[torch.Tensor] = None, out_dtype=None, skip_mod: int = 0) -> torch.Tensor:
    a, w = _gpu(a, name="a"), _gpu(w, a.dtype, "w")
    M, K = a.shape
    N = w.shape[0]
    assert w.shape[1] == K
    if bias is not None:
        bias = _gpu(bias, torch.float32, "bias")
    if epilogue == L.EPI_RESID:
        assert out is not None and out.dtype == torch.float32 and out.is_contiguous()
    elif out is None:
        out = torch.empty(M, N, dtype=out_dtype or a.dtype, device=a.device)
    L.check(L.lib().vtc_gemm(a.data_ptr(), w.data_ptr(), bias.data_ptr() if bias is not None else None, out.data_ptr(),
                             M, N, K, _TDT[a.dtype], epilogue, _TDT[out.dtype], skip_mod, _stream()), "vtc_gemm")
    return out


@on_device
def gemm_resid_layernorm(a: torch.Tensor, w: torch.Tensor, bias: Optional[torch.Tensor], out: torch.Tensor, ln_g: torch.Tensor,
                         ln_b: torch.Tensor, skip_mod: int = 0, ln_out: Optional[torch.Tensor] = None) -> torch.Tensor:
    a, w = _gpu(a, name="a"), _gpu(w, a.dtype, "w")
    M, K = a.shape
    N = w.shape[0]
    assert out.dtype == torch.float32 and out.shape == (M, N) and out.is_contiguous()
    lib = L.lib()
    if not lib.vtc_gemm_resid_layernorm_supported(M, N, K, _TDT[a.dtype]):
        raise ValueError(f"gemm_resid_layernorm: unsupported problem M={M} N={N} K={K} {a.dtype}")
    if ln_out is None:
        ln_out = torch.empty(M, N, dtype=a.dtype, device=a.device)
    ws = workspace(lib.vtc_gemm_resid_layernorm_workspace_bytes(M), a.device)
    L.check(lib.vtc_gemm_resid_layernorm(a.data_ptr(), w.data_ptr(), bias.data_ptr() if bias is not None else None, out.data_ptr(), M, N, K,
                                         _TDT[a.dtype], skip_mod, _gpu(ln_g, torch.float32).data_ptr(), _gpu(ln_b, torch.float32).data_ptr(),
                                         ln_out.data_ptr(), ws.data_ptr(), ws.numel(), _stream()), "vtc_gemm_resid_layernorm")
    return ln_out


@on_device
def layernorm(x: torch.Tensor, g: torch.Tensor, b: torch.Tensor, out_dtype=torch.float32, rows: Optional[int] = None,
              row_index: Optional[torch.Tensor] = None, row_mul: int = 1) -> torch.Tensor:
    x = _gpu(x, torch.float32, "x")
    width = x.shape[-1]
    n = rows if rows is not None else (row_index.numel() if row_index is not None else x.numel() // width)
    y = torch.empty(n, width, dtype=out_dtype, device=x.device)
    ri = _gpu(row_index, torch.int32, "row_index").data_ptr() if row_index is not None else None
    L.check(L.lib().vtc_layernorm(x.data_ptr(), _gpu(g, torch.float32).data_ptr(), _gpu(b, torch.float32).data_ptr(),
                                  y.data_ptr(), n, width, _TDT[out_dtype], ri, row_mul, _stream()), "vtc_layernorm")
    return y


@on_device
def attention(qkv: torch.Tensor, n_seq: int, L_: int, heads: int, causal: bool = False, s2: int = 1, a0: int = 0,
              a1: Optional[int] = None, a2: int = 0, a3: int = 0, pstride: int = 1, cls_out: Optional[torch.Tensor] = None,
              out: Optional[torch.Tensor] = None) -> torch.Tensor:
    qkv = _gpu(qkv, name="qkv")
    rows, w3 = qkv.shape
    W = w3 // 3
    assert W == heads * 64
    if a1 is None:
        a1 = L_
    if out is None:
        out = torch.zeros(rows, W, dtype=qkv.dtype, device=qkv.device)
    L.check(L.lib().vtc_attention(qkv.data_ptr(), out.data_ptr(), cls_out.data_ptr() if cls_out is not None else None,
                                  n_seq, L_, heads, int(causal), s2, a0, a1, a2, a3, pstride, _TDT[qkv.dtype], _stream()),
            "vtc_attention")
    return out


@on_device
def single_query_attention(qkv: torch.Tensor, q: torch.Tensor, n_out: int, L_: int, heads: int, s2: int = 1, a0: int = 0,
                           a1: Optional[int] = None, a2: int = 0, a3: int = 0, pstride: int = 1, eot: Optional[torch.Tensor] = None,
                           offs: Optional[torch.Tensor] = None, ctx: int = 0) -> torch.Tensor:
    qkv, q = _gpu(qkv, name="qkv"), _gpu(q, qkv.dtype, "q")
    W = qkv.shape[1] // 3
    assert W == heads * 64 and q.shape[1] == W
    if a1 is None:
        a1 = L_
    out = torch.empty(n_out, W, dtype=torch.float32, device=qkv.device)
    eot_p = _gpu(eot, torch.int32, "eot").data_ptr() if eot is not None else None
    offs_p = _gpu(offs, torch.int32, "offs").data_ptr() if offs is not None else None
    L.check(L.lib().vtc_single_query_attention(qkv.data_ptr(), q.data_ptr(), out.data_ptr(), n_out, L_, heads, s2, a0, a1, a2, a3, pstride,
                                               eot_p, offs_p, ctx, _TDT[qkv.dtype], _stream()), "vtc_single_query_attention")
    return out


_RESIZE_PLANS: dict = {}


def _resize_plan(in_h: int, in_w: int, size: int, device) -> torch.Tensor:
    key = (device, in_h, in_w, size)
    plan = _RESIZE_PLANS.get(key)
    if plan is None:
        lib = L.lib()
        nbytes = lib.vtc_resize_plan_bytes(in_h, in_w, size)
        host = torch.empty(max(nbytes, 4) // 4, dtype=torch.int32)
        L.check(lib.vtc_resize_plan(in_h, in_w, size, host.data_ptr(), nbytes), "vtc_resize_plan")
        if len(_RESIZE_PLANS) >= 256:
            _RESIZE_PLANS.clear()
        plan = _RESIZE_PLANS[key] = host.to(device)
    return plan


def clip_resize_crop(frames: torch.Tensor, size: int = 224, layout: str = "hwc", out: Optional[torch.Tensor] = None) -> torch.Tensor:
    if layout not in ("hwc", "chw"):
        raise ValueError(f"clip_resize_crop: layout {layout!r} (\"hwc\" or \"chw\")")
    if not isinstance(frames, torch.Tensor) or frames.dtype != torch.uint8:
        raise ValueError(f"clip_resize_crop: uint8 frames expected, got {getattr(frames, 'dtype', type(frames))}")
    if frames.dim() not in (3, 4, 5):
        raise ValueError(f"clip_resize_crop: frames of rank 3, 4 or 5 expected ([..., H, W, 3] or [..., 3, H, W]), got {tuple(frames.shape)}")
    lead = tuple(frames.shape[:-3])
    ch, (in_h, in_w) = (frames.shape[-1], frames.shape[-3:-1]) if layout == "hwc" else (frames.shape[-3], frames.shape[-2:])
    if ch != 3:
        raise ValueError(f"clip_resize_crop: 3 channels expected in layout {layout!r}, got shape {tuple(frames.shape)}")
    size = int(size)
    if size <= 0 or size % 16 or L.lib().vtc_resize_plan_bytes(int(in_h), int(in_w), size) == 0:
        raise ValueError(f"clip_resize_crop: size={size} must be a positive multiple of 16 (at most 1024) and the frame edges "
                         f"({in_h} x {in_w}) within [1, 8192]")
    n = 1
    for d in lead:
        n *= int(d)
    if n < 1:
        raise ValueError(f"clip_resize_crop: no frames in shape {tuple(frames.shape)}")
    if out is not None and (out.dtype != torch.uint8 or tuple(out.shape) != lead + (3, size, size) or not out.is_contiguous()
                            or out.device != frames.device or out.data_ptr() % 16):
        raise ValueError(f"clip_resize_crop: out must be a contiguous, 16-byte aligned uint8 tensor of shape {lead + (3, size, size)} on {frames.device}")
    return _clip_resize_crop(frames, n, int(in_h), int(in_w), size, 0 if layout == "hwc" else 1, lead, out)


@on_device
def _clip_resize_crop(frames, n, in_h, in_w, size, layout, lead, out):
    frames = _gpu(frames, torch.uint8, "frames")
    plan = _resize_plan(in_h, in_w, size, frames.device)
    if out is None:
        out = torch.empty(lead + (3, size, size), dtype=torch.uint8, device=frames.device)
    L.check(L.lib().vtc_resize_crop_u8(frames.data_ptr(), n, in_h, in_w, layout, plan.data_ptr(), size, out.data_ptr(), _stream()),
            "vtc_resize_crop_u8")
    return out


@on_device
def normalize_rows(x: torch.Tensor) -> torch.Tensor:
    x = _gpu(x, torch.float32, "x")
    out = torch.empty_like(x)
    L.check(L.lib().vtc_normalize_rows(x.data_ptr(), out.data_ptr(), x.shape[0], x.shape[1], _stream()), "vtc_normalize_rows")
    return out


@on_device
def mean_groups(x: torch.Tensor, group: int) -> torch.Tensor:
    x = _gpu(x, torch.float32, "x")
    n, d = x.shape
    assert n % group == 0
    out = torch.empty(n // group, d, dtype=torch.float32, device=x.device)
    L.check(L.lib().vtc_mean_groups(x.data_ptr(), out.data_ptr(), n // group, group, d, _stream()), "vtc_mean_groups")
    return out


@on_device
def mean_head_groups(a: torch.Tensor, b: torch.Tensor, group: int) -> torch.Tensor:
    a, b = _gpu(a, torch.float32, "a"), _gpu(b, torch.float32, "b")
    n, d = a.shape
    assert b.shape == (n * group, d)
    out = torch.empty(n, d, dtype=torch.float32, device=a.device)
    L.check(L.lib().vtc_mean_head_groups(a.data_ptr(), b.data_ptr(), out.data_ptr(), n, group, d, _stream()), "vtc_mean_head_groups")
    return out


@on_device
def pack_tokens(tokens: torch.Tensor, offsets: torch.Tensor, ctx: int = 77, sot: int = 49406, eot: int = 49407) -> torch.Tensor:
    tokens, offsets = _gpu(tokens, torch.int32, "tokens"), _gpu(offsets, torch.int32, "offsets")
    n = offsets.numel() - 1
    ids = torch.empty(n, ctx, dtype=torch.int64, device=offsets.device)
    L.check(L.lib().vtc_pack_tokens(tokens.data_ptr(), offsets.data_ptr(), n, ctx, sot, eot, ids.data_ptr(), _stream()), "vtc_pack_tokens")
    return ids


@on_device
def segment_mean(x: torch.Tensor, offsets: torch.Tensor) -> torch.Tensor:
    x = _gpu(x, torch.float32, "x")
    offsets = _gpu(offsets, torch.int32, "offsets")
    n = offsets.numel() - 1
    out = torch.empty(n, x.shape[1], dtype=torch.float32, device=x.device)
    L.check(L.lib().vtc_segment_mean(x.data_ptr(), offsets.data_ptr(), out.data_ptr(), n, x.shape[1], _stream()), "vtc_segment_mean")
    return out


@on_device
def normalize_rows2(x: torch.Tensor, y: torch.Tensor, flag: Optional[torch.Tensor] = None):
    x, y = _gpu(x, torch.float32, "x"), _gpu(y, torch.float32, "y")
    assert x.dim() == 2 and y.dim() == 2 and x.shape[1] == y.shape[1]
    ox, oy = torch.empty_like(x), torch.empty_like(y)
    L.check(L.lib().vtc_normalize_rows2(x.data_ptr(), ox.data_ptr(), x.shape[0], y.data_ptr(), oy.data_ptr(), y.shape[0], x.shape[1],
                                        flag.data_ptr() if flag is not None else None, _stream()), "vtc_normalize_rows2")
    return ox, oy


def nonfinite_flag2(a: torch.Tensor, b: torch.Tensor, flag: torch.Tensor) -> torch.Tensor:
    a, b = _gpu(a, torch.float32, "embeddings"), _gpu(b, torch.float32, "embeddings")
    with torch.cuda.device(a.device):
        L.check(L.lib().vtc_nonfinite_flag2(a.data_ptr(), a.numel(), b.data_ptr(), b.numel(), flag.data_ptr(), _stream()), "vtc_nonfinite_flag2")
    return flag


def nonfinite_bits(a: torch.Tensor, b: torch.Tensor) -> int:
    a = _gpu(a, torch.float32, "embeddings")
    return int(nonfinite_flag2(a, b, torch.zeros(1, dtype=torch.int32, device=a.device)).item())


@on_device
def similarity(v: torch.Tensor, t: torch.Tensor, logit_scale: torch.Tensor) -> torch.Tensor:
    v, t = _gpu(v, torch.float32, "v"), _gpu(t, torch.float32, "t")
    ls = _gpu(logit_scale.detach().reshape(1), torch.float32, "logit_scale")
    sim = torch.empty(v.shape[0], t.shape[0], dtype=torch.float32, device=v.device)
    L.check(L.lib().vtc_similarity(v.data_ptr(), t.data_ptr(), v.shape[0], t.shape[0], v.shape[1], ls.data_ptr(),
                                   sim.data_ptr(), _stream()), "vtc_similarity")
    return sim


@on_device
def clip_loss(sim: torch.Tensor) -> torch.Tensor:
    sim = _gpu(sim, torch.float32, "sim")
    n = sim.shape[0]
    assert sim.shape == (n, n)
    ws = workspace(L.lib().vtc_clip_loss_workspace_bytes(n), sim.device)
    loss = torch.empty((), dtype=torch.float32, device=sim.device)
    L.check(L.lib().vtc_clip_loss(sim.data_ptr(), n, loss.data_ptr(), ws.data_ptr(), ws.numel(), _stream()), "vtc_clip_loss")
    return loss


@on_device
def l2_topk(gallery: torch.Tensor, queries: torch.Tensor, depth: int, precision: int = L.SWEEP_EXACT,
            rows_per_block: int = 0, return_dists: bool = True, ws: Optional[torch.Tensor] = None):
    gallery, queries = _gpu(gallery, torch.float32, "gallery"), _gpu(queries, torch.float32, "queries")
    ng, d = gallery.shape
    nq = queries.shape[0]
    ws = _ws_for(ws, L.lib().vtc_l2_topk_workspace_bytes(ng, nq, d, precision, rows_per_block), gallery.device)
    ids = torch.empty(nq, depth, dtype=torch.int64, device=gallery.device)
    dists = torch.empty(nq, depth, dtype=torch.float32, device=gallery.device) if return_dists else None
    L.check(L.lib().vtc_l2_topk(gallery.data_ptr(), queries.data_ptr(), ng, nq, d, depth, precision, rows_per_block,
                                ids.data_ptr(), dists.data_ptr() if dists is not None else None, ws.data_ptr(), ws.numel(),
                                _stream()), "vtc_l2_topk")
    return ids, dists


@on_device
def l2_topk_bidir(a: torch.Tensor, b: torch.Tensor, depth: int, precision: int = L.SWEEP_EXACT, rows_per_block: int = 0,
                  return_dists: bool = True, ws: Optional[torch.Tensor] = None):
    a, b = _gpu(a, torch.float32, "a"), _gpu(b, torch.float32, "b")
    na, d = a.shape
    nb = b.shape[0]
    ws = _ws_for(ws, L.lib().vtc_l2_topk_bidir_workspace_bytes(na, nb, d, precision, rows_per_block), a.device)
    ids1 = torch.empty(nb, depth, dtype=torch.int64, device=a.device)
    ids2 = torch.empty(na, depth, dtype=torch.int64, device=a.device)
    d1 = torch.empty(nb, depth, dtype=torch.float32, device=a.device) if return_dists else None
    d2 = torch.empty(na, depth, dtype=torch.float32, device=a.device) if return_dists else None
    L.check(L.lib().vtc_l2_topk_bidir(a.data_ptr(), b.data_ptr(), na, nb, d, depth, precision, rows_per_block,
                                      ids1.data_ptr(), d1.data_ptr() if d1 is not None else None,
                                      ids2.data_ptr(), d2.data_ptr() if d2 is not None else None,
                                      ws.data_ptr(), ws.numel(), _stream()), "vtc_l2_topk_bidir")
    return ids1, d1, ids2, d2


SEARCH_MAX_QUERIES = 64


@on_device
def l2_search(gallery: torch.Tensor, queries: torch.Tensor, depth: int, id_base: int = 0, return_dists: bool = True,
              ws: Optional[torch.Tensor] = None, live: Optional[torch.Tensor] = None):
    gallery, queries = _gpu(gallery, torch.float32, "gallery"), _gpu(queries, torch.float32, "queries")
    ng, d = gallery.shape
    nq = queries.shape[0]
    if queries.shape[1] != d:
        raise ValueError(f"l2_search: gallery rows have {d} columns, queries {queries.shape[1]}")
    if live is not None:
        live = _gpu(live, torch.int32, "live")
        if live.device != gallery.device or tuple(live.shape) != ((ng + 31) // 32,):
            raise ValueError(f"l2_search: live must be int32 [{(ng + 31) // 32}] on {gallery.device} (one bit per gallery row), got "
                             f"{tuple(live.shape)} on {live.device}")
    need = L.lib().vtc_l2_search_workspace_bytes(ng, nq, d, depth)
    if ws is None:
        ws = workspace(need, gallery.device)
    elif need and (ws.numel() < need or ws.device != gallery.device):
        raise ValueError(f"l2_search: the workspace passed holds {ws.numel()} bytes on {ws.device}, the call needs {need} on {gallery.device}")
    ids = torch.empty(nq, depth, dtype=torch.int64, device=gallery.device)
    dists = torch.empty(nq, depth, dtype=torch.float32, device=gallery.device) if return_dists else None
    bits = torch.zeros(1, dtype=torch.int32, device=gallery.device)
    tail = (int(id_base), ids.data_ptr(), dists.data_ptr() if dists is not None else None, bits.data_ptr(), ws.data_ptr(), ws.numel(), _stream())
    if live is None:
        L.check(L.lib().vtc_l2_search(gallery.data_ptr(), queries.data_ptr(), ng, nq, d, depth, *tail), "vtc_l2_search")
    else:
        L.check(L.lib().vtc_l2_search_masked(gallery.data_ptr(), queries.data_ptr(), live.data_ptr(), ng, nq, d, depth, *tail),
                "vtc_l2_search_masked")
    return ids, dists, bits


@on_device
def row_mask_pack(flags: torch.Tensor, and_mask: Optional[torch.Tensor] = None) -> torch.Tensor:
    if flags.dtype == torch.bool:
        flags = flags.view(torch.uint8) if flags.is_contiguous() else flags.contiguous().view(torch.uint8)
    flags = _gpu(flags, torch.uint8, "flags")
    if flags.dim() != 1 or flags.shape[0] < 1:
        raise ValueError(f"row_mask_pack: flags must be [n] with n >= 1, got {tuple(flags.shape)}")
    n = flags.shape[0]
    if and_mask is not None:
        and_mask = _gpu(and_mask, torch.int32, "and_mask")
        if and_mask.device != flags.device or tuple(and_mask.shape) != ((n + 31) // 32,):
            raise ValueError(f"row_mask_pack: and_mask must be int32 [{(n + 31) // 32}] on {flags.device}, got {tuple(and_mask.shape)} on "
                             f"{and_mask.device}")
    words = torch.empty((n + 31) // 32, dtype=torch.int32, device=flags.device)
    L.check(L.lib().vtc_row_mask_pack(flags.data_ptr(), n, and_mask.data_ptr() if and_mask is not None else None, words.data_ptr(), _stream()),
            "vtc_row_mask_pack")
    return words


def l2_search_workspace_bytes(n_gallery: int, n_queries: int, d: int, depth: int) -> int:
    return int(L.lib().vtc_l2_search_workspace_bytes(int(n_gallery), int(n_queries), int(d), int(depth)))


def search_dists64(ws: torch.Tensor, n_queries: int, depth: int) -> torch.Tensor:
    return ws[:n_queries * depth * 8].view(torch.float64).view(n_queries, depth)


@on_device
def l2_search_part(gallery: torch.Tensor, queries: torch.Tensor, depth: int, id_base: int = 0, live: Optional[torch.Tensor] = None):
    ng, d = gallery.shape
    nq = queries.shape[0]
    ws = workspace(l2_search_workspace_bytes(ng, nq, d, depth), gallery.device)
    ids, _, bits = l2_search(gallery, queries, depth, id_base, return_dists=False, ws=ws, live=live)
    return ids, search_dists64(ws, nq, depth), bits


@on_device
def l2_search_merge(ids_parts: torch.Tensor, dists64_parts: torch.Tensor, return_dists: bool = True):
    ids_parts, dists64_parts = _gpu(ids_parts, torch.int64, "ids_parts"), _gpu(dists64_parts, torch.float64, "dists64_parts")
    if ids_parts.dim() != 3 or dists64_parts.shape != ids_parts.shape:
        raise ValueError(f"l2_search_merge: [parts, queries, depth] lists expected, got {tuple(ids_parts.shape)} and {tuple(dists64_parts.shape)}")
    n_parts, nq, depth = ids_parts.shape
    ids = torch.empty(nq, depth, dtype=torch.int64, device=ids_parts.device)
    dists = torch.empty(nq, depth, dtype=torch.float32, device=ids_parts.device) if return_dists else None
    L.check(L.lib().vtc_l2_search_merge(ids_parts.data_ptr(), dists64_parts.data_ptr(), n_parts, nq, depth, ids.data_ptr(),
                                        dists.data_ptr() if dists is not None else None, _stream()), "vtc_l2_search_merge")
    return ids, dists


@on_device
def l2_search_grouped(gallery: torch.Tensor, queries: torch.Tensor, groups: torch.Tensor, depth: int, id_base: int = 0,
                      return_dists: bool = True, ws: Optional[torch.Tensor] = None, live: Optional[torch.Tensor] = None):
    gallery, queries = _gpu(gallery, torch.float32, "gallery"), _gpu(queries, torch.float32, "queries")
    groups = _gpu(groups, torch.int32, "groups")
    ng, d = gallery.shape
    nq = queries.shape[0]
    if queries.shape[1] != d:
        raise ValueError(f"l2_search_grouped: gallery rows have {d} columns, queries {queries.shape[1]}")
    if groups.device != gallery.device or tuple(groups.shape) != (ng,):
        raise ValueError(f"l2_search_grouped: groups must be int32 [{ng}] on {gallery.device} (one id per gallery row), got "
                         f"{tuple(groups.shape)} on {groups.device}")
    if live is not None:
        live = _gpu(live, torch.int32, "live")
        if live.device != gallery.device or tuple(live.shape) != ((ng + 31) // 32,):
            raise ValueError(f"l2_search_grouped: live must be int32 [{(ng + 31) // 32}] on {gallery.device} (one bit per gallery row), got "
                             f"{tuple(live.shape)} on {live.device}")
    need = L.lib().vtc_l2_search_grouped_workspace_bytes(ng, nq, d, depth)
    if ws is None:
        ws = workspace(need, gallery.device)
    elif need and (ws.numel() < need or ws.device != gallery.device):
        raise ValueError(f"l2_search_grouped: the workspace passed holds {ws.numel()} bytes on {ws.device}, the call needs {need} on "
                         f"{gallery.device}")
    ids = torch.empty(nq, depth, dtype=torch.int64, device=gallery.device)
    out_groups = torch.empty(nq, depth, dtype=torch.int32, device=gallery.device)
    dists = torch.empty(nq, depth, dtype=torch.float32, device=gallery.device) if return_dists else None
    bits = torch.zeros(1, dtype=torch.int32, device=gallery.device)
    L.check(L.lib().vtc_l2_search_grouped(gallery.data_ptr(), queries.data_ptr(), live.data_ptr() if live is not None else None,
                                          groups.data_ptr(), ng, nq, d, depth, int(id_base), ids.data_ptr(), out_groups.data_ptr(),
                                          dists.data_ptr() if dists is not None else None, bits.data_ptr(), ws.data_ptr(), ws.numel(),
                                          _stream()), "vtc_l2_search_grouped")
    return ids, out_groups, dists, bits


def l2_search_grouped_workspace_bytes(n_gallery: int, n_queries: int, d: int, depth: int) -> int:
    return int(L.lib().vtc_l2_search_grouped_workspace_bytes(int(n_gallery), int(n_queries), int(d), int(depth)))


@on_device
def l2_search_grouped_part(gallery: torch.Tensor, queries: torch.Tensor, groups: torch.Tensor, depth: int, id_base: int = 0,
                           live: Optional[torch.Tensor] = None):
    ng, d = gallery.shape
    nq = queries.shape[0]
    ws = workspace(l2_search_grouped_workspace_bytes(ng, nq, d, depth), gallery.device)
    ids, out_groups, _, bits = l2_search_grouped(gallery, queries, groups, depth, id_base, return_dists=False, ws=ws, live=live)
    return ids, out_groups, search_dists64(ws, nq, depth), bits


@on_device
def l2_search_merge_grouped(ids_parts: torch.Tensor, dists64_parts: torch.Tensor, groups_parts: torch.Tensor, return_dists: bool = True):
    ids_parts, dists64_parts = _gpu(ids_parts, torch.int64, "ids_parts"), _gpu(dists64_parts, torch.float64, "dists64_parts")
    groups_parts = _gpu(groups_parts, torch.int32, "groups_parts")
    if ids_parts.dim() != 3 or dists64_parts.shape != ids_parts.shape or groups_parts.shape != ids_parts.shape:
        raise ValueError(f"l2_search_merge_grouped: [parts, queries, depth] lists expected, got {tuple(ids_parts.shape)}, "
                         f"{tuple(dists64_parts.shape)} and {tuple(groups_parts.shape)}")
    n_parts, nq, depth = ids_parts.shape
    ids = torch.empty(nq, depth, dtype=torch.int64, device=ids_parts.device)
    out_groups = torch.empty(nq, depth, dtype=torch.int32, device=ids_parts.device)
    dists = torch.empty(nq, depth, dtype=torch.float32, device=ids_parts.device) if return_dists else None
    L.check(L.lib().vtc_l2_search_merge_grouped(ids_parts.data_ptr(), dists64_parts.data_ptr(), groups_parts.data_ptr(), n_parts, nq, depth,
                                                ids.data_ptr(), out_groups.data_ptr(), dists.data_ptr() if dists is not None else None,
                                                _stream()), "vtc_l2_search_merge_grouped")
    return ids, out_groups, dists


def pad_search_part(ids: torch.Tensor, dists64: torch.Tensor, depth: int):
    short = depth - ids.shape[1]
    if short <= 0:
        return ids, dists64
    return (torch.nn.functional.pad(ids, (0, short), value=-1), torch.nn.functional.pad(dists64, (0, short), value=float("inf")))


def sweep_shard_supported(n_total: int, n_local: int, depth: int) -> bool:
    return bool(L.lib().vtc_l2_sweep_shard_supported(int(n_total), int(n_local), int(depth)))


def sweep_row_block() -> int:
    return int(L.lib().vtc_l2_sweep_row_block())


@on_device
def sweep_shard_rows(a_all: torch.Tensor, b_local: torch.Tensor, depth: int, nblk_pad: int, ws: Optional[torch.Tensor] = None):
    a_all, b_local = _gpu(a_all, torch.float32, "a_all"), _gpu(b_local, torch.float32, "b_local")
    n, d = a_all.shape
    nl = b_local.shape[0]
    ws = _ws_for(ws, L.lib().vtc_l2_sweep_shard_workspace_bytes(n, nl, d), a_all.device)
    ids = torch.empty(nl, depth, dtype=torch.int64, device=a_all.device)
    planes = torch.empty(4, nblk_pad, n, dtype=torch.int32, device=a_all.device)
    L.check(L.lib().vtc_l2_sweep_shard_rows(a_all.data_ptr(), b_local.data_ptr(), n, nl, d, depth, ids.data_ptr(), None,
                                            planes.data_ptr(), nblk_pad, ws.data_ptr(), ws.numel(), _stream()),
            "vtc_l2_sweep_shard_rows")
    return ids, planes


@on_device
def sweep_shard_cols(b_all: torch.Tensor, a_local: torch.Tensor, depth: int, planes: torch.Tensor, src_base: torch.Tensor,
                     ws: Optional[torch.Tensor] = None):
    b_all, a_local = _gpu(b_all, torch.float32, "b_all"), _gpu(a_local, torch.float32, "a_local")
    planes, src_base = _gpu(planes, torch.int32, "planes"), _gpu(src_base, torch.int32, "src_base")
    n, d = b_all.shape
    nl = a_local.shape[0]
    n_src, four, nblk_pad, nl2 = planes.shape
    if four != 4 or nl2 != nl or src_base.numel() != n_src:
        raise ValueError(f"sweep_shard_cols: planes {tuple(planes.shape)} / src_base {tuple(src_base.shape)} do not match n_local={nl}")
    ws = _ws_for(ws, L.lib().vtc_l2_sweep_shard_workspace_bytes(n, nl, d), b_all.device)
    ids = torch.empty(nl, depth, dtype=torch.int64, device=b_all.device)
    L.check(L.lib().vtc_l2_sweep_shard_cols(b_all.data_ptr(), a_local.data_ptr(), n, nl, d, depth, planes.data_ptr(), n_src,
                                            nblk_pad, src_base.data_ptr(), ids.data_ptr(), None, ws.data_ptr(), ws.numel(),
                                            _stream()), "vtc_l2_sweep_shard_cols")
    return ids


def recall_bidir_supported(n: int, d: int) -> bool:
    return bool(L.lib().vtc_l2_recall_bidir_supported(int(n), int(d)))


@on_device
def recall_bidir(a: torch.Tensor, b: torch.Tensor, k_vals: Sequence[int], ws: Optional[torch.Tensor] = None,
                 hits: Optional[torch.Tensor] = None) -> torch.Tensor:
    a, b = _gpu(a, torch.float32, "a"), _gpu(b, torch.float32, "b")
    n, d = a.shape
    assert b.shape == (n, d) and 1 <= len(k_vals) <= 4
    if hits is None:
        hits = torch.zeros(2, len(k_vals), dtype=torch.int64, device=a.device)
    assert hits.shape == (2, len(k_vals)) and hits.is_contiguous() and hits.dtype == torch.int64
    ws = _ws_for(ws, L.lib().vtc_l2_recall_bidir_workspace_bytes(n, d), a.device)
    ks = _k_array(k_vals)
    L.check(L.lib().vtc_l2_recall_bidir(a.data_ptr(), b.data_ptr(), n, d, ks, len(k_vals), hits[0].data_ptr(), hits[1].data_ptr(),
                                        ws.data_ptr(), ws.numel(), _stream()), "vtc_l2_recall_bidir")
    return hits


def _rank_call(name, head, size_args, n_a, n_b, device, rows_per_block, reach_capacity, ws):
    lib = L.lib()
    ws = _ws_for(ws, getattr(lib, name + "_workspace_bytes")(*size_args, rows_per_block, reach_capacity), device)
    rank_a = torch.empty(max(n_a, 1), dtype=torch.int64, device=device)
    rank_b = torch.empty(n_b, dtype=torch.int64, device=device)
    bits = torch.empty(1, dtype=torch.int32, device=device)
    L.check(getattr(lib, name)(*head, rows_per_block, reach_capacity, rank_a.data_ptr(), rank_b.data_ptr(), bits.data_ptr(), ws.data_ptr(),
                               ws.numel(), _stream()), name)
    return rank_a[:n_a], rank_b, bits


@on_device
def rank_bidir(a: torch.Tensor, b: torch.Tensor, rows_per_block: int = 0, reach_capacity: int = 0, ws: Optional[torch.Tensor] = None):
    a, b = _gpu(a, torch.float32, "a"), _gpu(b, torch.float32, "b")
    n, d = a.shape
    if b.shape != (n, d):
        raise ValueError(f"rank_bidir: paired rows expected, got {tuple(a.shape)} and {tuple(b.shape)}")
    return _rank_call("vtc_l2_rank_bidir", (a.data_ptr(), b.data_ptr(), n, d), (n, d), n, n, a.device, rows_per_block, reach_capacity, ws)


def rank_shard(a_all: torch.Tensor, b_all: torch.Tensor, row_base: int, n_local: int, rows_per_block: int = 0, reach_capacity: int = 0,
               ws: Optional[torch.Tensor] = None):
    if a_all.dim() != 2 or a_all.shape[0] < 1 or b_all.shape != a_all.shape:
        raise ValueError(f"rank_shard: paired rows expected, got {tuple(a_all.shape)} and {tuple(b_all.shape)}")
    n = a_all.shape[0]
    row_base, n_local = int(row_base), int(n_local)
    if row_base < 0 or n_local < 0 or row_base + n_local > n:
        raise ValueError(f"rank_shard: window row_base={row_base}, n_local={n_local} must lie in [0, n_total={n}]")
    return _rank_shard(a_all, b_all, row_base, n_local, rows_per_block, reach_capacity, ws)


@on_device
def _rank_shard(a_all, b_all, row_base, n_local, rows_per_block, reach_capacity, ws):
    a_all, b_all = _gpu(a_all, torch.float32, "a_all"), _gpu(b_all, torch.float32, "b_all")
    n, d = a_all.shape
    return _rank_call("vtc_l2_rank_shard", (a_all.data_ptr(), b_all.data_ptr(), n, row_base, n_local, d), (n, n_local, d), n_local, n,
                      a_all.device, rows_per_block, reach_capacity, ws)


def check_offsets(offsets, n: int, m: int, allow_empty: bool = True):
    import numpy as np
    if isinstance(offsets, torch.Tensor):
        offsets = offsets.detach().cpu().numpy()
    off = np.asarray(offsets)
    if off.ndim != 1 or off.shape[0] != n + 1:
        raise ValueError(f"offsets: expected {n + 1} entries for {n} videos, got shape {tuple(off.shape)}")
    if off.dtype.kind not in "iu":
        if off.dtype.kind != "f" or not np.array_equal(off, np.floor(off)):
            raise ValueError(f"offsets: integers expected, got dtype {off.dtype}")
    off = off.astype(np.int64)
    if off[0] != 0 or off[-1] != m:
        raise ValueError(f"offsets: must start at 0 and end at the number of captions {m}, got {int(off[0])} .. {int(off[-1])}")
    steps = np.diff(off)
    if (steps < 0).any():
        raise ValueError(f"offsets: must be non-decreasing (first descent after video {int(np.flatnonzero(steps < 0)[0])})")
    if not allow_empty and (steps == 0).any():
        raise ValueError(f"offsets: video {int(np.flatnonzero(steps == 0)[0])} has no caption")
    return off


def rank_grouped(a: torch.Tensor, b: torch.Tensor, offsets, rows_per_block: int = 0, reach_capacity: int = 0,
                 ws: Optional[torch.Tensor] = None):
    if a.dim() != 2 or b.dim() != 2 or a.shape[1] != b.shape[1] or a.shape[0] < 1 or b.shape[0] < 1:
        raise ValueError(f"rank_grouped: a [n, d] and b [m, d] expected, got {tuple(a.shape)} and {tuple(b.shape)}")
    off = check_offsets(offsets, a.shape[0], b.shape[0])
    return _rank_grouped(a, b, off, rows_per_block, reach_capacity, ws)


@on_device
def _rank_grouped(a, b, off, rows_per_block, reach_capacity, ws):
    a, b = _gpu(a, torch.float32, "a"), _gpu(b, torch.float32, "b")
    (n, d), m = a.shape, b.shape[0]
    off_dev = torch.from_numpy(off.astype("int32")).to(a.device)
    return _rank_call("vtc_l2_rank_grouped", (a.data_ptr(), b.data_ptr(), off_dev.data_ptr(), n, m, d), (n, m, d), m, n, a.device,
                      rows_per_block, reach_capacity, ws)


def rank_grouped_vunit(a: torch.Tensor, b: torch.Tensor, offsets, rows_per_block: int = 0, reach_capacity: int = 0,
                       ws: Optional[torch.Tensor] = None):
    if a.dim() != 2 or b.dim() != 2 or a.shape[1] != b.shape[1] or a.shape[0] < 1 or b.shape[0] < 1:
        raise ValueError(f"rank_grouped_vunit: a [n, d] and b [m, d] expected, got {tuple(a.shape)} and {tuple(b.shape)}")
    off = check_offsets(offsets, a.shape[0], b.shape[0])
    return _rank_grouped_vunit(a, b, off, rows_per_block, reach_capacity, ws)


@on_device
def _rank_grouped_vunit(a, b, off, rows_per_block, reach_capacity, ws):
    a, b = _gpu(a, torch.float32, "a"), _gpu(b, torch.float32, "b")
    (n, d), m = a.shape, b.shape[0]
    lib = L.lib()
    off_dev = torch.from_numpy(off.astype("int32")).to(a.device)
    ws = _ws_for(ws, lib.vtc_l2_rank_grouped_vunit_workspace_bytes(n, m, d, rows_per_block, reach_capacity), a.device)
    rank_a = torch.empty(m, dtype=torch.int64, device=a.device)
    rank_b = torch.empty(n, dtype=torch.int64, device=a.device)
    rank_v = torch.empty(n, dtype=torch.int64, device=a.device)
    bits = torch.empty(1, dtype=torch.int32, device=a.device)
    L.check(lib.vtc_l2_rank_grouped_vunit(a.data_ptr(), b.data_ptr(), off_dev.data_ptr(), n, m, d, rows_per_block, reach_capacity,
                                          rank_a.data_ptr(), rank_b.data_ptr(), rank_v.data_ptr(), bits.data_ptr(), ws.data_ptr(),
                                          ws.numel(), _stream()), "vtc_l2_rank_grouped_vunit")
    return rank_a, rank_b, rank_v, bits


def rank_kappa(d: int) -> float:
    return float(L.lib().vtc_l2_rank_kappa(int(d)))


def rank_sweep_stats(ws: torch.Tensor) -> dict:
    w = ws[:88].view(torch.int64).cpu().tolist()
    return {"in_reach": (w[0], w[1]), "in_reach_max": (w[2], w[3]), "brute_force_owners": (w[4], w[5]),
            "vunit_in_reach": w[8], "vunit_in_reach_max": w[9], "vunit_brute_force_owners": w[10]}


def split_recall_counters(hits_host: torch.Tensor):
    h = hits_host.numpy()
    return torch.from_numpy(h & (L.RECALL_NONFINITE - 1)), bool((h >> 40).any())


def recall_planes(k_vals: Sequence[int], n_total: int) -> int:
    ks = _k_array(k_vals)
    return int(L.lib().vtc_l2_recall_planes(ks, len(k_vals), int(n_total)))


def recall_shard_supported(n_total: int, n_local: int, d: int) -> bool:
    return bool(L.lib().vtc_l2_recall_shard_supported(int(n_total), int(n_local), int(d)))


@on_device
def recall_shard_rows(a_all: torch.Tensor, b_local: torch.Tensor, row_base: int, k_vals: Sequence[int], nblk_pad: int, hits: torch.Tensor,
                      ws: Optional[torch.Tensor] = None) -> torch.Tensor:
    a_all, b_local = _gpu(a_all, torch.float32, "a_all"), _gpu(b_local, torch.float32, "b_local")
    n, d = a_all.shape
    nl = b_local.shape[0]
    assert hits.shape == (len(k_vals),) and hits.dtype == torch.int64 and hits.is_contiguous() and hits.device == a_all.device
    ws = _ws_for(ws, L.lib().vtc_l2_sweep_shard_workspace_bytes(n, nl, d), a_all.device)
    ks = _k_array(k_vals)
    planes = torch.empty(L.lib().vtc_l2_recall_planes(ks, len(k_vals), n), nblk_pad, n, dtype=torch.int32, device=a_all.device)
    L.check(L.lib().vtc_l2_recall_shard_rows(a_all.data_ptr(), b_local.data_ptr(), n, nl, int(row_base), d, ks, len(k_vals), hits.data_ptr(),
                                             planes.data_ptr(), nblk_pad, ws.data_ptr(), ws.numel(), _stream()), "vtc_l2_recall_shard_rows")
    return planes


@on_device
def recall_shard_cols(b_all: torch.Tensor, a_local: torch.Tensor, row_base: int, k_vals: Sequence[int], planes: torch.Tensor,
                      src_bounds: torch.Tensor, hits: torch.Tensor, ws: Optional[torch.Tensor] = None) -> torch.Tensor:
    b_all, a_local = _gpu(b_all, torch.float32, "b_all"), _gpu(a_local, torch.float32, "a_local")
    planes, src_bounds = _gpu(planes, torch.int32, "planes"), _gpu(src_bounds, torch.int32, "src_bounds")
    n, d = b_all.shape
    nl = a_local.shape[0]
    n_src, npl, nblk_pad, nl2 = planes.shape
    ks = _k_array(k_vals)
    if npl != L.lib().vtc_l2_recall_planes(ks, len(k_vals), n) or nl2 != nl or src_bounds.numel() != n_src + 1:
        raise ValueError(f"recall_shard_cols: planes {tuple(planes.shape)} / src_bounds {tuple(src_bounds.shape)} do not match n_local={nl}, "
                         f"k_vals={list(k_vals)}")
    assert hits.shape == (len(k_vals),) and hits.dtype == torch.int64 and hits.is_contiguous() and hits.device == b_all.device
    ws = _ws_for(ws, L.lib().vtc_l2_sweep_shard_workspace_bytes(n, nl, d), b_all.device)
    L.check(L.lib().vtc_l2_recall_shard_cols(b_all.data_ptr(), a_local.data_ptr(), n, nl, int(row_base), d, ks, len(k_vals), planes.data_ptr(),
                                             n_src, nblk_pad, src_bounds.data_ptr(), hits.data_ptr(), ws.data_ptr(), ws.numel(), _stream()),
            "vtc_l2_recall_shard_cols")
    return hits


@on_device
def recall_hits_pair(ids_a: torch.Tensor, ids_b: torch.Tensor, k_vals: Sequence[int], target_offset: int, hits: torch.Tensor) -> torch.Tensor:
    ids_a, ids_b = _gpu(ids_a, torch.int64, "ids_a"), _gpu(ids_b, torch.int64, "ids_b")
    assert ids_a.shape == ids_b.shape and hits.shape[0] == 2 and hits.is_contiguous()
    nq, depth = ids_a.shape
    ks = _k_array(k_vals)
    L.check(L.lib().vtc_recall_hits_pair(ids_a.data_ptr(), ids_b.data_ptr(), nq, depth, int(target_offset), ks, len(k_vals),
                                         hits[0].data_ptr(), hits[1].data_ptr(), _stream()), "vtc_recall_hits_pair")
    return hits


@on_device
def recall_hits(ids: torch.Tensor, k_vals: Sequence[int], target_offset: int = 0,
                hits: Optional[torch.Tensor] = None) -> torch.Tensor:
    ids = _gpu(ids, torch.int64, "ids")
    nq, depth = ids.shape
    if hits is None:
        hits = torch.zeros(len(k_vals), dtype=torch.int64, device=ids.device)
    ks = _k_array(k_vals)
    L.check(L.lib().vtc_recall_hits(ids.data_ptr(), nq, depth, int(target_offset), ks, len(k_vals), hits.data_ptr(), _stream()),
            "vtc_recall_hits")
    return hits


@on_device
def nonfinite_flag(x: torch.Tensor, flag: torch.Tensor) -> torch.Tensor:
    x = _gpu(x, torch.float32, "x")
    L.check(L.lib().vtc_nonfinite_flag(x.data_ptr(), x.numel(), flag.data_ptr(), _stream()), "vtc_nonfinite_flag")
    return flag


def _f32(t: torch.Tensor, name: str) -> torch.Tensor:
    return _gpu(t, torch.float32, name)


@on_device
def transpose(x: torch.Tensor, out: Optional[torch.Tensor] = None) -> torch.Tensor:
    x = _f32(x, "x")
    r, c = x.shape
    out = torch.empty(c, r, dtype=torch.float32, device=x.device) if out is None else out
    L.check(L.lib().vtc_transpose_f32(x.data_ptr(), out.data_ptr(), r, c, _stream()), "vtc_transpose_f32")
    return out


@on_device
def colsum(x: torch.Tensor, out: Optional[torch.Tensor] = None) -> torch.Tensor:
    x = _f32(x, "x")
    out = torch.empty(x.shape[1], dtype=torch.float32, device=x.device) if out is None else out
    L.check(L.lib().vtc_colsum_f32(x.data_ptr(), out.data_ptr(), x.shape[0], x.shape[1], _stream()), "vtc_colsum_f32")
    return out


@on_device
def layernorm_bwd(x: torch.Tensor, gamma: torch.Tensor, dy: torch.Tensor, dx: Optional[torch.Tensor] = None, accumulate_dx: bool = False,
                  dgamma: Optional[torch.Tensor] = None, dbeta: Optional[torch.Tensor] = None):
    x, gamma, dy = _f32(x, "x"), _f32(gamma, "gamma"), _f32(dy, "dy")
    if dx is None:
        assert not accumulate_dx
        dx = torch.empty_like(x)
    dgamma = torch.empty_like(gamma) if dgamma is None else dgamma
    dbeta = torch.empty_like(gamma) if dbeta is None else dbeta
    L.check(L.lib().vtc_layernorm_bwd(x.data_ptr(), gamma.data_ptr(), dy.data_ptr(), dx.data_ptr(), dgamma.data_ptr(), dbeta.data_ptr(),
                                      x.shape[0], x.shape[1], int(accumulate_dx), _stream()), "vtc_layernorm_bwd")
    return dx, dgamma, dbeta


@on_device
def attention_small_bwd(qkv: torch.Tensor, dout: torch.Tensor, n_seq: int, L_: int, heads: int, out: Optional[torch.Tensor] = None) -> torch.Tensor:
    qkv, dout = _f32(qkv, "qkv"), _f32(dout, "dout")
    out = torch.empty_like(qkv) if out is None else out
    L.check(L.lib().vtc_attention_small_bwd(qkv.data_ptr(), dout.data_ptr(), out.data_ptr(), n_seq, L_, heads, _stream()), "vtc_attention_small_bwd")
    return out


@on_device
def quickgelu(x: torch.Tensor, dy: Optional[torch.Tensor] = None, out: Optional[torch.Tensor] = None) -> torch.Tensor:
    x = _f32(x, "x")
    out = torch.empty_like(x) if out is None else out
    L.check(L.lib().vtc_quickgelu(x.data_ptr(), _f32(dy, "dy").data_ptr() if dy is not None else None, out.data_ptr(), x.numel(), _stream()),
            "vtc_quickgelu")
    return out


@on_device
def normalize_rows_bwd(x: torch.Tensor, dy: torch.Tensor, out: Optional[torch.Tensor] = None) -> torch.Tensor:
    x, dy = _f32(x, "x"), _f32(dy, "dy")
    out = torch.empty_like(x) if out is None else out
    L.check(L.lib().vtc_normalize_rows_bwd(x.data_ptr(), dy.data_ptr(), out.data_ptr(), x.shape[0], x.shape[1], _stream()), "vtc_normalize_rows_bwd")
    return out


@on_device
def clip_loss_bwd(sim: torch.Tensor, out: Optional[torch.Tensor] = None, ws: Optional[torch.Tensor] = None) -> torch.Tensor:
    sim = _f32(sim, "sim")
    n = sim.shape[0]
    assert sim.shape == (n, n)
    out = torch.empty_like(sim) if out is None else out
    ws = torch.empty(4 * n, dtype=torch.float32, device=sim.device) if ws is None else ws
    L.check(L.lib().vtc_clip_loss_bwd(sim.data_ptr(), n, out.data_ptr(), ws.data_ptr(), ws.numel() * ws.element_size(), _stream()), "vtc_clip_loss_bwd")
    return out


@on_device
def adam_step(p: torch.Tensor, g: torch.Tensor, m: torch.Tensor, v: torch.Tensor, vmax: Optional[torch.Tensor], lr: float, beta1: float,
              beta2: float, eps: float, step: int, amsgrad: bool) -> torch.Tensor:
    p, g, m, v = _f32(p, "p"), _f32(g, "g"), _f32(m, "m"), _f32(v, "v")
    L.check(L.lib().vtc_adam_step(p.data_ptr(), g.data_ptr(), m.data_ptr(), v.data_ptr(), _f32(vmax, "vmax").data_ptr() if vmax is not None else None,
                                  p.numel(), lr, beta1, beta2, eps, int(step), int(amsgrad), _stream()), "vtc_adam_step")
    return p


@on_device
def axpby(x: torch.Tensor, y: Optional[torch.Tensor], a: float, b: float, out: Optional[torch.Tensor] = None) -> torch.Tensor:
    x = _f32(x, "x")
    out = torch.empty_like(x) if out is None else out
    L.check(L.lib().vtc_axpby(out.data_ptr(), x.data_ptr(), _f32(y, "y").data_ptr() if y is not None else None, a, b, x.numel(), _stream()), "vtc_axpby")
    return out


@on_device
def scale_rows(x: torch.Tensor, s: torch.Tensor, group: int = 1) -> torch.Tensor:
    x, s = _f32(x, "x"), _f32(s, "s")
    L.check(L.lib().vtc_scale_rows(x.data_ptr(), s.data_ptr(), x.shape[0], x.shape[1], group, _stream()), "vtc_scale_rows")
    return x
```

Before: 8954 pairs/s.

## Fold K/V projections into query-side attention for the last-block single-query tail

```diff
diff --git a/include/vtc_hip.h b/include/vtc_hip.h
--- a/include/vtc_hip.h
+++ b/include/vtc_hip.h
@@ -214,6 +214,13 @@
 int vtc_single_query_attention(const void *qkv, const void *q, float *out, int n_out, int L, int heads, int s2, int a0, int a1, int a2,
                                int a3, int pstride, const int *eot, const int *offs, int ctx, int dtype, void *stream);
 
+int vtc_query_fold(const void *q, const void *qkv_wf, void *u, float *a, int n_q, int heads, int dtype, void *stream);
+int vtc_stream_attention(const void *xb, const float *stat, const void *u, const float *a, float *z, float *m, int n_q, int L, int heads,
+                         int s2, int a0, int a1, int a2, int a3, int pstride, const int *eot, const int *offs, int ctx, int dtype,
+                         void *stream);
+int vtc_value_fold(const float *z, const float *m, const void *qkv_wf, const float *qkv_s, const float *qkv_c, void *out, int n_q, int heads,
+                   int dtype, void *stream);
+
 int vtc_transpose_f32(const float *x, float *y, int rows, int cols, void *stream);
 int vtc_colsum_f32(const float *x, float *out, int rows, int cols, void *stream);
 int vtc_layernorm_bwd(const float *x, const float *gamma, const float *dy, float *dx, float *dgamma, float *dbeta, int rows,
diff --git a/vtc_amd/_lib.py b/vtc_amd/_lib.py
--- a/vtc_amd/_lib.py
+++ b/vtc_amd/_lib.py
@@ -80,6 +80,9 @@
     "vtc_mean_head_groups": (C.c_int, [fp, fp, fp, C.c_int, C.c_int, C.c_int, vp]),
     "vtc_pack_tokens": (C.c_int, [vp, vp, C.c_int, C.c_int, C.c_int, C.c_int, vp, vp]),
     "vtc_single_query_attention": (C.c_int, [vp, vp, fp] + [C.c_int] * 9 + [vp, vp, C.c_int, C.c_int, vp]),
+    "vtc_query_fold": (C.c_int, [vp, vp, vp, fp, C.c_int, C.c_int, C.c_int, vp]),
+    "vtc_stream_attention": (C.c_int, [vp, fp, vp, fp, fp, fp] + [C.c_int] * 9 + [vp, vp, C.c_int, C.c_int, vp]),
+    "vtc_value_fold": (C.c_int, [fp, fp, vp, fp, fp, vp, C.c_int, C.c_int, C.c_int, vp]),
     "vtc_segment_mean": (C.c_int, [fp, ip, fp, C.c_int, C.c_int, vp]),
     "vtc_similarity": (C.c_int, [fp, fp, C.c_int, C.c_int, C.c_int, fp, fp, vp]),
     "vtc_clip_loss_workspace_bytes": (C.c_size_t, [C.c_int]),
diff --git a/vtc_amd/csrc/common.h b/vtc_amd/csrc/common.h
--- a/vtc_amd/csrc/common.h
+++ b/vtc_amd/csrc/common.h
@@ -253,5 +253,11 @@
 int launch_single_query_attention(const void *qkv, const void *q, float *out, int n_out, int L, int heads, int s2, int a0, int a1, int a2,
                                   int a3, int pstride, const int *eot, const int *offs, int ctx, int dtype, hipStream_t stream);
 int launch_mean_cast(const float *x, void *out, int n, int F, int W, int dtype, hipStream_t stream);
+bool stream_attention_supported(int W, int heads, int dtype);
+int launch_query_fold(const void *q, const void *qkv_wf, void *u, float *a, int n_q, int heads, int dtype, hipStream_t stream);
+int launch_stream_attention(const void *xb, const float *stat, const void *u, const float *a, float *z, float *m, int n_q, int L, int heads, int s2,
+                            int a0, int a1, int a2, int a3, int pstride, const int *eot, const int *offs, int ctx, int dtype, hipStream_t stream);
+int launch_value_fold(const float *z, const float *m, const void *qkv_wf, const float *qkv_s, const float *qkv_c, void *out, int n_q, int heads,
+                      int dtype, hipStream_t stream);
 int launch_attention(const void *qkv, void *out, float *cls_out, int n_seq, int L, int heads, int causal, int s2,
                      int a0, int a1, int a2, int a3, int pstride, int dtype, hipStream_t stream);
diff --git a/vtc_amd/csrc/stream_attn.hip b/vtc_amd/csrc/stream_attn.hip
--- /dev/null
+++ b/vtc_amd/csrc/stream_attn.hip
@@ -0,0 +1,418 @@
+#include "common.h"
+
+namespace {
+
+template <typename T> __device__ __forceinline__ f32x4 mfma_k32(const uint4 &a, const uint4 &b, f32x4 acc);
+template <> __device__ __forceinline__ f32x4 mfma_k32<bf16_t>(const uint4 &a, const uint4 &b, f32x4 acc) {
+  return __builtin_amdgcn_mfma_f32_16x16x32_bf16(__builtin_bit_cast(bf16x8, a), __builtin_bit_cast(bf16x8, b), acc, 0, 0, 0);
+}
+template <> __device__ __forceinline__ f32x4 mfma_k32<f16_t>(const uint4 &a, const uint4 &b, f32x4 acc) {
+  return __builtin_amdgcn_mfma_f32_16x16x32_f16(__builtin_bit_cast(f16x8, a), __builtin_bit_cast(f16x8, b), acc, 0, 0, 0);
+}
+
+template <typename T>
+__device__ __forceinline__ void unpack8(const uint4 &raw, float (&f)[8]) {
+  const unsigned w[4] = {raw.x, raw.y, raw.z, raw.w};
+#pragma unroll
+  for (int e = 0; e < 4; ++e) {
+    f[2 * e] = up16<T>((unsigned short)(w[e] & 0xFFFFu));
+    f[2 * e + 1] = up16<T>((unsigned short)(w[e] >> 16));
+  }
+}
+
+constexpr int QF_QB = 8;
+template <typename T, int NC>
+__global__ __launch_bounds__(256) void query_fold_kernel(const unsigned short *__restrict__ q, const unsigned short *__restrict__ wk,
+                                                         unsigned short *__restrict__ u, float *__restrict__ a, int n_q, int heads, int W) {
+  __shared__ __align__(16) float qs[64][QF_QB];
+  __shared__ float red[4][QF_QB];
+  const int tid = threadIdx.x, lane = tid & 63, wave = tid >> 6;
+  const int h = blockIdx.y, q0 = blockIdx.x * QF_QB;
+  for (int i = tid; i < QF_QB * 64; i += 256) {
+    const int qi = q0 + (i >> 6);
+    qs[i & 63][i >> 6] = qi < n_q ? 0.125f * up16<T>(q[(size_t)qi * W + h * 64 + (i & 63)]) : 0.f;
+  }
+  __syncthreads();
+  float acc[QF_QB][NC];
+#pragma unroll
+  for (int b = 0; b < QF_QB; ++b)
+#pragma unroll
+    for (int i = 0; i < NC; ++i) acc[b][i] = 0.f;
+  const unsigned short *wrow = wk + (size_t)h * 64 * W;
+#pragma unroll 4
+  for (int d = 0; d < 64; ++d) {
+    float wv[NC];
+#pragma unroll
+    for (int i = 0; i < NC; ++i) {
+      const int c = min(tid + 256 * i, W - 1);
+      wv[i] = up16<T>(wrow[(size_t)d * W + c]);
+    }
+    const float4 q0v = *reinterpret_cast<const float4 *>(&qs[d][0]), q1v = *reinterpret_cast<const float4 *>(&qs[d][4]);
+    const float qv[QF_QB] = {q0v.x, q0v.y, q0v.z, q0v.w, q1v.x, q1v.y, q1v.z, q1v.w};
+#pragma unroll
+    for (int b = 0; b < QF_QB; ++b)
+#pragma unroll
+      for (int i = 0; i < NC; ++i) acc[b][i] = fmaf(qv[b], wv[i], acc[b][i]);
+  }
+#pragma unroll
+  for (int b = 0; b < QF_QB; ++b) {
+    const int qi = q0 + b;
+    if (qi >= n_q) break;
+    unsigned short *uh = u + ((size_t)qi * heads + h) * 2 * W;
+    float s = 0.f;
+#pragma unroll
+    for (int i = 0; i < NC; ++i) {
+      const int c = tid + 256 * i;
+      if (c < W) {
+        const unsigned short hi = cvt16<T>(acc[b][i]);
+        const unsigned short lo = cvt16<T>(acc[b][i] - up16<T>(hi));
+        uh[c] = hi;
+        uh[W + c] = lo;
+        s += up16<T>(hi) + up16<T>(lo);
+      }
+    }
+    s = wave_sum(s);
+    if (lane == 0) red[wave][b] = s;
+  }
+  __syncthreads();
+  if (tid < QF_QB && q0 + tid < n_q) a[(size_t)(q0 + tid) * heads + h] = (red[0][tid] + red[1][tid]) + (red[2][tid] + red[3][tid]);
+}
+
+struct StreamAttnParams {
+  const char *xb;
+  const float2 *stat;
+  const unsigned short *u;
+  const float *a;
+  float *z, *m;
+  int n_q, F, L, a0, a1, a2, a3, pstride;
+  const int *eot, *offs;
+  int ctx, CH;
+};
+constexpr int SA_ROW_PAD = 16;
+__host__ __device__ constexpr int sa_head_stride(int H) { return H < 4 ? 4 : (H + 3) / 4 * 4; }
+__host__ __device__ inline size_t sa_lds_bytes(int W, int CH) {
+  const int CHP = (CH + 15) / 16 * 16;
+  return (size_t)CH * (W * 2 + SA_ROW_PAD) + (size_t)CHP * sa_head_stride(W / 64) * 4 + (size_t)CHP * 8 + 5 * 16 * 4;
+}
+
+template <typename T, int W>
+__global__ __launch_bounds__(256) void stream_attn_kernel(const StreamAttnParams p) {
+  constexpr int H = W / 64, NC = (W + 255) / 256, RS = W * 2 + SA_ROW_PAD, HS = sa_head_stride(H), CPR = W / 8, LB = 10, KG = W >= 256 ? 8 : 4;
+  extern __shared__ __align__(16) char sa_smem[];
+  const int CH = p.CH, CHP = (CH + 15) / 16 * 16;
+  char *tile = sa_smem;
+  float *sc = reinterpret_cast<float *>(sa_smem + (size_t)CH * RS);
+  float2 *st = reinterpret_cast<float2 *>(sc + (size_t)CHP * HS);
+  float *hs = reinterpret_cast<float *>(st + CHP);
+  float *h_max = hs, *h_sum = hs + 16, *h_alpha = hs + 32, *h_m = hs + 48, *h_mq = hs + 64;
+  const int tid = threadIdx.x, lane = tid & 63, wave = tid >> 6, g = lane >> 4, l15 = lane & 15;
+  const int qi = blockIdx.x;
+  const float invF = 1.0f / (float)p.F;
+
+  float zq[H][NC], zs[H][NC];
+#pragma unroll
+  for (int h = 0; h < H; ++h)
+#pragma unroll
+    for (int i = 0; i < NC; ++i) zq[h][i] = 0.f;
+  if (tid < 16) h_mq[tid] = 0.f;
+
+  const unsigned short *u_hi = p.u + ((size_t)qi * H + (l15 < H ? l15 : H - 1)) * 2 * W + 8 * g;
+  const unsigned short *u_lo = u_hi + W;
+  const float a_h = l15 < H ? p.a[(size_t)qi * H + l15] : 0.f;
+
+  for (int f = 0; f < p.F; ++f) {
+    const int o = qi * p.F + f;
+    long base;
+    int first, pstride, L;
+    if (p.eot) {
+      base = p.offs ? (long)p.offs[o] : (long)o * p.ctx;
+      L = min(p.eot[o] - (int)base + 1, p.ctx);
+      first = 1; pstride = 1;
+    } else {
+      base = (long)qi * p.a1 + (long)f * p.a2 + p.a0;
+      first = 1 + f * p.a3; pstride = p.pstride; L = p.L;
+    }
+    L = min(max(L, 1), 4096);
+    auto row_of = [&](int tok) -> long { return tok == 0 ? base : base + first + (long)(tok - 1) * pstride; };
+#pragma unroll
+    for (int h = 0; h < H; ++h)
+#pragma unroll
+      for (int i = 0; i < NC; ++i) zs[h][i] = 0.f;
+    if (tid < 16) { h_max[tid] = -INFINITY; h_sum[tid] = 0.f; h_m[tid] = 0.f; }
+
+    for (int r0 = 0; r0 < L; r0 += CH) {
+      const int n = min(CH, L - r0);
+      __syncthreads();
+      for (int i0 = tid; i0 < n * CPR; i0 += 256 * LB) {
+        uint4 v[LB];
+#pragma unroll
+        for (int k = 0; k < LB; ++k) {
+          const int i = i0 + 256 * k, r = i / CPR, c = i - r * CPR;
+          v[k] = make_uint4(0u, 0u, 0u, 0u);
+          if (i < n * CPR) v[k] = *reinterpret_cast<const uint4 *>(p.xb + ((size_t)row_of(r0 + r) * W + c * 8) * 2);
+        }
+#pragma unroll
+        for (int k = 0; k < LB; ++k) {
+          const int i = i0 + 256 * k, r = i / CPR, c = i - r * CPR;
+          if (i < n * CPR) *reinterpret_cast<uint4 *>(tile + (size_t)r * RS + c * 16) = v[k];
+        }
+      }
+      for (int i = tid; i < n; i += 256) st[i] = p.stat[row_of(r0 + i)];
+      __syncthreads();
+
+      for (int t = wave; t * 16 < n; t += 4) {
+        const char *ap = tile + (size_t)min(t * 16 + l15, n - 1) * RS + 16 * g;
+        f32x4 acc = {0.f, 0.f, 0.f, 0.f};
+        for (int kg = 0; kg < W; kg += 32 * KG) {
+          uint4 bh[KG], bl[KG];
+#pragma unroll
+          for (int k = 0; k < KG; ++k) {
+            bh[k] = *reinterpret_cast<const uint4 *>(u_hi + kg + 32 * k);
+            bl[k] = *reinterpret_cast<const uint4 *>(u_lo + kg + 32 * k);
+          }
+#pragma unroll
+          for (int k = 0; k < KG; ++k) {
+            const uint4 av = *reinterpret_cast<const uint4 *>(ap + (kg + 32 * k) * 2);
+            acc = mfma_k32<T>(av, bh[k], acc);
+            acc = mfma_k32<T>(av, bl[k], acc);
+          }
+        }
+        if (l15 < H) {
+#pragma unroll
+          for (int i = 0; i < 4; ++i) {
+            const int row = t * 16 + 4 * g + i;
+            if (row < n) {
+              const float2 s = st[row];
+              sc[row * HS + l15] = s.y * (acc[i] - s.x * a_h);
+            }
+          }
+        }
+      }
+      __syncthreads();
+
+      for (int h = wave; h < H; h += 4) {
+        float mx = -INFINITY;
+        for (int j = lane; j < n; j += 64) mx = fmaxf(mx, sc[j * HS + h]);
+        mx = wave_max(mx);
+        const float m_old = h_max[h], m_new = fmaxf(m_old, mx);
+        const float alpha = __expf(m_old - m_new);
+        float ps = 0.f, pm = 0.f;
+        for (int j = lane; j < n; j += 64) {
+          const float e = __expf(sc[j * HS + h] - m_new);
+          const float2 s = st[j];
+          const float w = e * s.y;
+          sc[j * HS + h] = w;
+          ps += e;
+          pm = fmaf(w, s.x, pm);
+        }
+        ps = wave_sum(ps);
+        pm = wave_sum(pm);
+        if (lane == 0) {
+          h_max[h] = m_new;
+          h_sum[h] = h_sum[h] * alpha + ps;
+          h_alpha[h] = alpha;
+          h_m[h] = h_m[h] * alpha + pm;
+        }
+      }
+      __syncthreads();
+
+#pragma unroll
+      for (int h = 0; h < H; ++h) {
+        const float al = h_alpha[h];
+#pragma unroll
+        for (int i = 0; i < NC; ++i) zs[h][i] *= al;
+      }
+      const char *col[NC];
+#pragma unroll
+      for (int i = 0; i < NC; ++i) col[i] = tile + min(tid + 256 * i, W - 1) * 2;
+#pragma unroll 4
+      for (int j = 0; j < n; ++j) {
+        float xv[NC];
+#pragma unroll
+        for (int i = 0; i < NC; ++i) xv[i] = up16<T>(*reinterpret_cast<const unsigned short *>(col[i] + j * RS));
+        float wv[HS];
+#pragma unroll
+        for (int h4 = 0; h4 < HS / 4; ++h4) {
+          const float4 w4 = *reinterpret_cast<const float4 *>(sc + j * HS + 4 * h4);
+          wv[4 * h4] = w4.x; wv[4 * h4 + 1] = w4.y; wv[4 * h4 + 2] = w4.z; wv[4 * h4 + 3] = w4.w;
+        }
+#pragma unroll
+        for (int h = 0; h < H; ++h)
+#pragma unroll
+          for (int i = 0; i < NC; ++i) zs[h][i] = fmaf(wv[h], xv[i], zs[h][i]);
+      }
+    }
+#pragma unroll
+    for (int h = 0; h < H; ++h) {
+      const float inv = invF / h_sum[h];
+#pragma unroll
+      for (int i = 0; i < NC; ++i) zq[h][i] = fmaf(zs[h][i], inv, zq[h][i]);
+    }
+    if (tid < H) h_mq[tid] += h_m[tid] * (invF / h_sum[tid]);
+    __syncthreads();
+  }
+#pragma unroll
+  for (int h = 0; h < H; ++h)
+#pragma unroll
+    for (int i = 0; i < NC; ++i) {
+      const int c = tid + 256 * i;
+      if (c < W) p.z[((size_t)qi * H + h) * W + c] = zq[h][i];
+    }
+  if (tid < H) p.m[(size_t)qi * H + tid] = h_mq[tid];
+}
+
+constexpr int VF_QB = 8;
+template <typename T>
+__global__ __launch_bounds__(256) void value_fold_kernel(const float *__restrict__ z, const float *__restrict__ m, const unsigned short *__restrict__ wv,
+                                                         const float *__restrict__ sv, const float *__restrict__ cv, unsigned short *__restrict__ out,
+                                                         int n_q, int heads, int W) {
+  extern __shared__ __align__(16) char vf_smem[];
+  float *zs = reinterpret_cast<float *>(vf_smem);
+  const int tid = threadIdx.x, h = blockIdx.y, q0 = blockIdx.x * VF_QB;
+  const int W4 = W / 4;
+  for (int i = tid; i < VF_QB * W4; i += 256) {
+    const int b = i / W4, c4 = i - b * W4, qi = q0 + b;
+    float4 v = make_float4(0.f, 0.f, 0.f, 0.f);
+    if (qi < n_q) v = *reinterpret_cast<const float4 *>(z + ((size_t)qi * heads + h) * W + c4 * 4);
+    reinterpret_cast<float4 *>(zs)[i] = v;
+  }
+  __syncthreads();
+  const int d = tid >> 2, part = tid & 3;
+  const unsigned short *wrow = wv + (size_t)(h * 64 + d) * W;
+  float acc[VF_QB];
+#pragma unroll
+  for (int b = 0; b < VF_QB; ++b) acc[b] = 0.f;
+  for (int ch = part; ch < W / 8; ch += 4) {
+    float wf[8];
+    unpack8<T>(*reinterpret_cast<const uint4 *>(wrow + ch * 8), wf);
+#pragma unroll
+    for (int b = 0; b < VF_QB; ++b) {
+      const float4 z0 = *reinterpret_cast<const float4 *>(zs + b * W + ch * 8);
+      const float4 z1 = *reinterpret_cast<const float4 *>(zs + b * W + ch * 8 + 4);
+      float s = acc[b];
+      s = fmaf(wf[0], z0.x, s); s = fmaf(wf[1], z0.y, s); s = fmaf(wf[2], z0.z, s); s = fmaf(wf[3], z0.w, s);
+      s = fmaf(wf[4], z1.x, s); s = fmaf(wf[5], z1.y, s); s = fmaf(wf[6], z1.z, s); s = fmaf(wf[7], z1.w, s);
+      acc[b] = s;
+    }
+  }
+#pragma unroll
+  for (int b = 0; b < VF_QB; ++b) {
+    acc[b] += __shfl_xor(acc[b], 1, 64);
+    acc[b] += __shfl_xor(acc[b], 2, 64);
+  }
+  if (part == 0) {
+    const float s_d = sv[h * 64 + d], c_d = cv[h * 64 + d];
+#pragma unroll
+    for (int b = 0; b < VF_QB; ++b) {
+      const int qi = q0 + b;
+      if (qi < n_q) out[(size_t)qi * W + h * 64 + d] = cvt16<T>(acc[b] - m[(size_t)qi * heads + h] * s_d + c_d);
+    }
+  }
+}
+
+template <typename T, int NC>
+void run_query_fold(const void *q, const void *wk, void *u, float *a, int n_q, int heads, int W, hipStream_t s) {
+  hipLaunchKernelGGL((query_fold_kernel<T, NC>), dim3(cdiv(n_q, QF_QB), heads), dim3(256), 0, s, (const unsigned short *)q,
+                     (const unsigned short *)wk, (unsigned short *)u, a, n_q, heads, W);
+}
+template <typename T>
+int launch_query_fold_t(const void *q, const void *wk, void *u, float *a, int n_q, int heads, int W, hipStream_t s) {
+  switch (cdiv(W, 256)) {
+    case 1: run_query_fold<T, 1>(q, wk, u, a, n_q, heads, W, s); break;
+    case 2: run_query_fold<T, 2>(q, wk, u, a, n_q, heads, W, s); break;
+    case 3: run_query_fold<T, 3>(q, wk, u, a, n_q, heads, W, s); break;
+    default: run_query_fold<T, 4>(q, wk, u, a, n_q, heads, W, s); break;
+  }
+  VTC_LAUNCH_CHECK("query_fold");
+  return 0;
+}
+
+constexpr int SA_LDS_TWO_PER_CU = 80 * 1024;
+template <typename T, int W>
+int run_stream_attn(const StreamAttnParams &p, hipStream_t s) {
+  static PerDeviceOnce attr;
+  if (ensure_dynamic_lds(attr, reinterpret_cast<const void *>(&stream_attn_kernel<T, W>), 160 * 1024, "stream_attention")) return 1;
+  hipLaunchKernelGGL((stream_attn_kernel<T, W>), dim3(p.n_q), dim3(256), sa_lds_bytes(W, p.CH), s, p);
+  VTC_LAUNCH_CHECK("stream_attention");
+  return 0;
+}
+template <typename T>
+int launch_stream_attn_t(const StreamAttnParams &p, int W, hipStream_t s) {
+  switch (W) {
+    case 128: return run_stream_attn<T, 128>(p, s);
+    case 256: return run_stream_attn<T, 256>(p, s);
+    case 512: return run_stream_attn<T, 512>(p, s);
+    case 768: return run_stream_attn<T, 768>(p, s);
+    case 1024: return run_stream_attn<T, 1024>(p, s);
+  }
+  VTC_CHECK(false, "stream_attention: width %d (128, 256, 512, 768 or 1024)", W);
+  return 1;
+}
+
+}
+
+bool stream_attention_supported(int W, int heads, int dtype) {
+  return (dtype == VTC_BF16 || dtype == VTC_F16) && W == heads * 64 && (W == 128 || W == 256 || W == 512 || W == 768 || W == 1024);
+}
+
+int launch_query_fold(const void *q, const void *qkv_wf, void *u, float *a, int n_q, int heads, int dtype, hipStream_t stream) {
+  const int W = heads * 64;
+  VTC_CHECK(n_q > 0 && heads > 0 && W <= 1024 && (dtype == VTC_BF16 || dtype == VTC_F16), "query_fold: n_q=%d heads=%d dtype=%d", n_q, heads, dtype);
+  const void *wk = (const char *)qkv_wf + (size_t)W * W * 2;
+  ProfScope prof(VTC_PROF_ATTN, 2.0 * W * W * (double)n_q, stream);
+  return dtype == VTC_F16 ? launch_query_fold_t<f16_t>(q, wk, u, a, n_q, heads, W, stream) : launch_query_fold_t<bf16_t>(q, wk, u, a, n_q, heads, W, stream);
+}
+
+int launch_stream_attention(const void *xb, const float *stat, const void *u, const float *a, float *z, float *m, int n_q, int L, int heads, int s2,
+                            int a0, int a1, int a2, int a3, int pstride, const int *eot, const int *offs, int ctx, int dtype, hipStream_t stream) {
+  const int W = heads * 64;
+  VTC_CHECK(n_q > 0 && s2 > 0 && (eot ? (ctx > 0 && s2 == 1) : L > 0), "stream_attention: bad sizes n_q=%d L=%d s2=%d ctx=%d", n_q, L, s2, ctx);
+  VTC_CHECK(stream_attention_supported(W, heads, dtype), "stream_attention: heads=%d dtype=%d unsupported", heads, dtype);
+  StreamAttnParams p;
+  p.xb = (const char *)xb; p.stat = (const float2 *)stat; p.u = (const unsigned short *)u; p.a = a; p.z = z; p.m = m;
+  p.n_q = n_q; p.F = s2; p.L = L; p.a0 = a0; p.a1 = a1; p.a2 = a2; p.a3 = a3; p.pstride = pstride;
+  p.eot = eot; p.offs = offs; p.ctx = ctx;
+  const int Lmax = eot ? ctx : L;
+  int CH = Lmax;
+  if (sa_lds_bytes(W, CH) > (size_t)SA_LDS_TWO_PER_CU) {
+    CH = 16;
+    while (CH + 16 < Lmax && sa_lds_bytes(W, CH + 16) <= (size_t)SA_LDS_TWO_PER_CU) CH += 16;
+  }
+  p.CH = CH;
+  ProfScope prof(VTC_PROF_ATTN, 4.0 * (eot ? 0.5 * ctx : L) * W * (double)n_q * s2 * heads, stream);
+  return dtype == VTC_F16 ? launch_stream_attn_t<f16_t>(p, W, stream) : launch_stream_attn_t<bf16_t>(p, W, stream);
+}
+
+int launch_value_fold(const float *z, const float *m, const void *qkv_wf, const float *qkv_s, const float *qkv_c, void *out, int n_q, int heads,
+                      int dtype, hipStream_t stream) {
+  const int W = heads * 64;
+  VTC_CHECK(n_q > 0 && heads > 0 && W <= 1024 && (dtype == VTC_BF16 || dtype == VTC_F16), "value_fold: n_q=%d heads=%d dtype=%d", n_q, heads, dtype);
+  const unsigned short *wv = (const unsigned short *)qkv_wf + (size_t)2 * W * W;
+  ProfScope prof(VTC_PROF_ATTN, 2.0 * W * W * (double)n_q, stream);
+  const dim3 grid(cdiv(n_q, VF_QB), heads);
+  const size_t shmem = (size_t)VF_QB * W * 4;
+  if (dtype == VTC_F16)
+    hipLaunchKernelGGL((value_fold_kernel<f16_t>), grid, dim3(256), shmem, stream, z, m, wv, qkv_s + 2 * W, qkv_c + 2 * W, (unsigned short *)out, n_q, heads, W);
+  else
+    hipLaunchKernelGGL((value_fold_kernel<bf16_t>), grid, dim3(256), shmem, stream, z, m, wv, qkv_s + 2 * W, qkv_c + 2 * W, (unsigned short *)out, n_q, heads, W);
+  VTC_LAUNCH_CHECK("value_fold");
+  return 0;
+}
+
+extern "C" int vtc_query_fold(const void *q, const void *qkv_wf, void *u, float *a, int n_q, int heads, int dtype, void *stream) {
+  VTC_CHECK(q && qkv_wf && u && a, "query_fold: null argument");
+  return launch_query_fold(q, qkv_wf, u, a, n_q, heads, dtype, (hipStream_t)stream);
+}
+
+extern "C" int vtc_stream_attention(const void *xb, const float *stat, const void *u, const float *a, float *z, float *m, int n_q, int L, int heads,
+                                    int s2, int a0, int a1, int a2, int a3, int pstride, const int *eot, const int *offs, int ctx, int dtype,
+                                    void *stream) {
+  VTC_CHECK(xb && stat && u && a && z && m, "stream_attention: null argument");
+  return launch_stream_attention(xb, stat, u, a, z, m, n_q, L, heads, s2, a0, a1, a2, a3, pstride, eot, offs, ctx, dtype, (hipStream_t)stream);
+}
+
+extern "C" int vtc_value_fold(const float *z, const float *m, const void *qkv_wf, const float *qkv_s, const float *qkv_c, void *out, int n_q, int heads,
+                              int dtype, void *stream) {
+  VTC_CHECK(z && m && qkv_wf && qkv_s && qkv_c && out, "value_fold: null argument");
+  return launch_value_fold(z, m, qkv_wf, qkv_s, qkv_c, out, n_q, heads, dtype, (hipStream_t)stream);
+}
diff --git a/vtc_amd/csrc/towers.hip b/vtc_amd/csrc/towers.hip
--- a/vtc_amd/csrc/towers.hip
+++ b/vtc_amd/csrc/towers.hip
@@ -201,13 +201,29 @@
   void *h = nullptr;
   void *big = nullptr;
   float *sq = nullptr;
+  void *uz = nullptr;
+  float *am = nullptr;
 };
-void plan_tail(Bump &b, Tail &t, int n, int W) {
+void plan_tail(Bump &b, Tail &t, int n, int W, bool stream_scratch) {
   t.x = (float *)b.take((size_t)n * W * 4);
   t.a = b.take((size_t)n * W * 4);
   t.h = b.take((size_t)n * W * 4);
   t.big = b.take((size_t)n * 4 * W * 4);
   t.sq = (float *)b.take((size_t)n * W * 4);
+  if (!stream_scratch) return;
+  t.uz = b.take((size_t)n * (W / 64) * W * 4);
+  t.am = (float *)b.take((size_t)2 * n * (W / 64) * 4);
+}
+inline bool stream_tail_path(const Act &a, LastBlock last, int heads, int dtype) {
+  return last == LastBlock::OneQueryPerSequence && a.fold.on && stream_attention_supported(a.W, heads, dtype);
+}
+int tail_stream_attention(Act &a, const vtc_block_w &b, Tail &t, int n, int L, int heads, int s2, int a1, int a3, int pstride, const int *eot,
+                          const int *offs, int ctx, int dtype) {
+  float *am = t.am, *m = t.am + (size_t)n * heads;
+  RUN(fold_enter(a, dtype));
+  RUN(launch_query_fold(t.big, b.qkv_wf, t.uz, am, n, heads, dtype, a.s));
+  RUN(launch_stream_attention(a.fold.xb, a.fold.stat, t.uz, am, (float *)t.uz, m, n, L, heads, s2, 0, a1, 0, a3, pstride, eot, offs, ctx, dtype, a.s));
+  return launch_value_fold((const float *)t.uz, m, b.qkv_wf, b.qkv_s, b.qkv_c, t.a, n, heads, dtype, a.s);
 }
 int gather_output_rows(Act &a, Tail &t, int n, const int *row_index, int row_mul) {
   RUN(fold_merge_rows(a, n, row_index, row_mul));
@@ -242,7 +258,7 @@
   v.cls_tmp = (float *)b.take((size_t)n_items * (F > P ? F : P) * W * 4);
   v.lnp = b.take((size_t)n_items * W * 4);
   plan_fold(b, v.a.fold, rows, W, dtype);
-  plan_tail(b, v.tail, n_items, W);
+  plan_tail(b, v.tail, n_items, W, dtype != VTC_F32 && W == w->heads * 64);
   v.total = b.off;
   return v;
 }
@@ -255,7 +271,7 @@
   Tail tail;
   size_t total;
 };
-TextWs plan_text(int rows_, int n_seq, int W, int dtype, void *ws, hipStream_t s = nullptr) {
+TextWs plan_text(int rows_, int n_seq, int W, int dtype, bool stream_scratch, void *ws, hipStream_t s = nullptr) {
   Bump b(ws);
   TextWs t;
   const size_t rows = (size_t)pad256(rows_);
@@ -267,7 +283,7 @@
   t.offs = (int *)b.take((size_t)(n_seq + 1) * 4);
   t.mdev = (int *)b.take(16);
   plan_fold(b, t.a.fold, rows, W, dtype);
-  plan_tail(b, t.tail, n_seq, W);
+  plan_tail(b, t.tail, n_seq, W, stream_scratch && dtype != VTC_F32);
   t.total = b.off;
   return t;
 }
@@ -344,6 +360,7 @@
   };
 
   const LastBlock last = last_block_path(w->flags, w->layers, v1);
+  const bool stream_tail = stream_tail_path(a, last, w->heads, dtype);
   for (int l = 0; l < w->layers; ++l) {
     const vtc_block_w &b = w->blocks[l];
     ProfRegion region(VTC_PROF_REGION_ATTN);
@@ -372,9 +389,13 @@
       case LastBlock::OneQueryPerSequence:
         if (tsf) RUN(time_branch(b));
         RUN(tail_query(a, b, v.tail, n_items, nullptr, T, dtype));
-        RUN(ln_proj(a, qkv_of(b), 3 * W, dtype, VTC_EPI_STORE, W, 2 * W));
-        RUN(launch_single_query_attention(a.big, v.tail.big, v.cls_tmp, n_items * F, 1 + P, w->heads, F, 0, T, 0, tsf ? 1 : 0, F, nullptr, nullptr, 0, dtype, s));
-        RUN(launch_mean_cast(v.cls_tmp, v.tail.a, n_items, F, W, dtype, s));
+        if (stream_tail) {
+          RUN(tail_stream_attention(a, b, v.tail, n_items, 1 + P, w->heads, F, T, tsf ? 1 : 0, F, nullptr, nullptr, 0, dtype));
+        } else {
+          RUN(ln_proj(a, qkv_of(b), 3 * W, dtype, VTC_EPI_STORE, W, 2 * W));
+          RUN(launch_single_query_attention(a.big, v.tail.big, v.cls_tmp, n_items * F, 1 + P, w->heads, F, 0, T, 0, tsf ? 1 : 0, F, nullptr, nullptr, 0, dtype, s));
+          RUN(launch_mean_cast(v.cls_tmp, v.tail.a, n_items, F, W, dtype, s));
+        }
         RUN(tail_finish(b, v.tail, n_items, W, dtype, s));
         break;
     }
@@ -390,7 +411,7 @@
 }
 
 extern "C" size_t vtc_text_workspace_bytes(const vtc_text_w *w, int n_seq, int dtype) {
-  return plan_text(n_seq * w->ctx, n_seq, w->width, dtype, nullptr).total;
+  return plan_text(n_seq * w->ctx, n_seq, w->width, dtype, w->width == w->heads * 64, nullptr).total;
 }
 
 namespace {
@@ -402,7 +423,7 @@
   VTC_CHECK(w->ctx <= 80, "%s: context %d > 80 unsupported", who, w->ctx);
   VTC_CHECK(w->width == w->heads * 64, "%s: head_dim must be 64", who);
   const int rows_host = kind == TextRows::HostOffsets ? total_rows : n_seq * w->ctx;
-  TextWs t = plan_text(rows_host, n_seq, W, dtype, ws, s);
+  TextWs t = plan_text(rows_host, n_seq, W, dtype, true, ws, s);
   VTC_CHECK(ws_bytes >= t.total, "%s: workspace too small (%zu < %zu)", who, ws_bytes, t.total);
   Act &a = t.a;
   const int *offs = seq_offsets;
@@ -413,6 +434,7 @@
   }
   fold_begin(a, w->blocks, w->layers, dtype, false, w->flags);
   const LastBlock last = last_block_path(w->flags, w->layers, false);
+  const bool stream_tail = stream_tail_path(a, last, w->heads, dtype);
   const bool ragged = kind != TextRows::Dense;
   const int dl0 = (dtype == VTC_BF16 && w->half_layers > 0) ? VTC_F16 : dtype;
   if (!ragged) {
@@ -441,10 +463,14 @@
         break;
       case LastBlock::OneQueryPerSequence:
         RUN(tail_query(a, b, t.tail, n_seq, t.eot, 1, dl));
-        RUN(ln_proj(a, qkv_of(b), 3 * W, dl, VTC_EPI_STORE, W, 2 * W));
-        RUN(launch_single_query_attention(a.big, t.tail.big, t.tail.sq, n_seq, 0, w->heads, 1, 0, 0, 0, 0, 1, t.eot,
-                                          kind == TextRows::Dense ? nullptr : offs, w->ctx, dl, s));
-        RUN(launch_mean_cast(t.tail.sq, t.tail.a, n_seq, 1, W, dl, s));
+        if (stream_tail) {
+          RUN(tail_stream_attention(a, b, t.tail, n_seq, 0, w->heads, 1, 0, 0, 1, t.eot, kind == TextRows::Dense ? nullptr : offs, w->ctx, dl));
+        } else {
+          RUN(ln_proj(a, qkv_of(b), 3 * W, dl, VTC_EPI_STORE, W, 2 * W));
+          RUN(launch_single_query_attention(a.big, t.tail.big, t.tail.sq, n_seq, 0, w->heads, 1, 0, 0, 0, 0, 1, t.eot,
+                                            kind == TextRows::Dense ? nullptr : offs, w->ctx, dl, s));
+          RUN(launch_mean_cast(t.tail.sq, t.tail.a, n_seq, 1, W, dl, s));
+        }
         RUN(tail_finish(b, t.tail, n_seq, W, dl, s));
         break;
       case LastBlock::OutputRowsAfterAttention: VTC_CHECK(false, "%s: last_block_path() chose the variant-1 video tower's path", who);
@@ -478,7 +504,7 @@
 }
 
 extern "C" size_t vtc_text_ragged_workspace_bytes(const vtc_text_w *w, int n_seq, int total_rows, int dtype) {
-  return plan_text(total_rows, n_seq, w->width, dtype, nullptr).total;
+  return plan_text(total_rows, n_seq, w->width, dtype, w->width == w->heads * 64, nullptr).total;
 }
 
 extern "C" int vtc_text_forward_ragged(const vtc_text_w *w, const int64_t *ids, int n_seq, const int *seq_offsets, int total_rows,
@@ -490,7 +516,7 @@
 }
 
 static size_t cam_ws_bytes(const vtc_cam_w *w, int B, int Lc, int dtype) {
-  TextWs t = plan_text(B * Lc, B, w->width, dtype, nullptr);
+  TextWs t = plan_text(B * Lc, B, w->width, dtype, false, nullptr);
   return t.total + align_up((size_t)B * w->width * 4, 256) + align_up(cam_fused_bar_bytes(), 256);
 }
 
@@ -508,7 +534,7 @@
   const int D = w->width, Lc = 1 + nc + na, rows = B * Lc;
   VTC_CHECK(w->heads >= 1 && w->width % w->heads == 0 && (w->width == w->heads * 64 || (w->width / w->heads <= 128 && Lc <= 16)),
             "cam_forward: head_dim %d / %d: 64, or <= 128 with at most 16 tokens per item", w->width, w->heads);
-  TextWs t = plan_text(rows, B, D, dtype, ws, s);
+  TextWs t = plan_text(rows, B, D, dtype, false, ws, s);
   Act &a = t.a;
   float *lin = (float *)((char *)ws + t.total);
   VTC_CHECK(ws_bytes >= cam_ws_bytes(w, B, Lc, dtype), "cam_forward: workspace too small");
diff --git a/vtc_amd/ops.py b/vtc_amd/ops.py
--- a/vtc_amd/ops.py
+++ b/vtc_amd/ops.py
@@ -144,6 +144,51 @@
     offs_p = _gpu(offs, torch.int32, "offs").data_ptr() if offs is not None else None
     L.check(L.lib().vtc_single_query_attention(qkv.data_ptr(), q.data_ptr(), out.data_ptr(), n_out, L_, heads, s2, a0, a1, a2, a3, pstride,
                                                eot_p, offs_p, ctx, _TDT[qkv.dtype], _stream()), "vtc_single_query_attention")
+    return out
+
+
+@on_device
+def query_fold(q: torch.Tensor, qkv_wf: torch.Tensor, heads: int):
+    q, qkv_wf = _gpu(q, name="q"), _gpu(qkv_wf, q.dtype, "qkv_wf")
+    n_q, W = q.shape
+    assert W == heads * 64 and qkv_wf.shape == (3 * W, W)
+    u = torch.empty(n_q, heads, 2, W, dtype=q.dtype, device=q.device)
+    a = torch.empty(n_q, heads, dtype=torch.float32, device=q.device)
+    L.check(L.lib().vtc_query_fold(q.data_ptr(), qkv_wf.data_ptr(), u.data_ptr(), a.data_ptr(), n_q, heads, _TDT[q.dtype], _stream()),
+            "vtc_query_fold")
+    return u, a
+
+
+@on_device
+def stream_attention(xb: torch.Tensor, stat: torch.Tensor, u: torch.Tensor, a: torch.Tensor, L_: int, heads: int, s2: int = 1,
+                     a0: int = 0, a1: Optional[int] = None, a2: int = 0, a3: int = 0, pstride: int = 1,
+                     eot: Optional[torch.Tensor] = None, offs: Optional[torch.Tensor] = None, ctx: int = 0):
+    xb, u = _gpu(xb, name="xb"), _gpu(u, xb.dtype, "u")
+    stat, a = _gpu(stat, torch.float32, "stat"), _gpu(a, torch.float32, "a")
+    W = xb.shape[1]
+    n_q = u.shape[0]
+    assert W == heads * 64 and u.shape == (n_q, heads, 2, W) and stat.shape == (xb.shape[0], 2) and a.shape == (n_q, heads)
+    if a1 is None:
+        a1 = L_
+    z = torch.empty(n_q, heads, W, dtype=torch.float32, device=xb.device)
+    m = torch.empty(n_q, heads, dtype=torch.float32, device=xb.device)
+    eot_p = _gpu(eot, torch.int32, "eot").data_ptr() if eot is not None else None
+    offs_p = _gpu(offs, torch.int32, "offs").data_ptr() if offs is not None else None
+    L.check(L.lib().vtc_stream_attention(xb.data_ptr(), stat.data_ptr(), u.data_ptr(), a.data_ptr(), z.data_ptr(), m.data_ptr(), n_q, L_, heads,
+                                         s2, a0, a1, a2, a3, pstride, eot_p, offs_p, ctx, _TDT[xb.dtype], _stream()), "vtc_stream_attention")
+    return z, m
+
+
+@on_device
+def value_fold(z: torch.Tensor, m: torch.Tensor, qkv_wf: torch.Tensor, qkv_s: torch.Tensor, qkv_c: torch.Tensor) -> torch.Tensor:
+    z, m = _gpu(z, torch.float32, "z"), _gpu(m, torch.float32, "m")
+    qkv_wf = _gpu(qkv_wf, name="qkv_wf")
+    n_q, heads, W = z.shape
+    assert W == heads * 64 and qkv_wf.shape == (3 * W, W) and qkv_wf.dtype in (torch.bfloat16, torch.float16)
+    out = torch.empty(n_q, W, dtype=qkv_wf.dtype, device=z.device)
+    L.check(L.lib().vtc_value_fold(z.data_ptr(), m.data_ptr(), qkv_wf.data_ptr(), _gpu(qkv_s, torch.float32, "qkv_s").data_ptr(),
+                                   _gpu(qkv_c, torch.float32, "qkv_c").data_ptr(), out.data_ptr(), n_q, heads, _TDT[qkv_wf.dtype], _stream()),
+            "vtc_value_fold")
     return out
 
 
```

Result: no change. 8953 pairs/s (-0.0%).
